# Ulixes-8/UNet-Implementations

Measured on AMD Instinct MI355X. Metric: images/sec (512x512, bs/GPU=8) Our_UNet train step, higher is better.
Workload: dtype f32; 1 GPU; Our_UNet 6-stage 3-class 512x512 bs=8/GPU fp32 train step (fwd + Dice/wCE loss + bwd + SGD-Nesterov), train mode, HIP conv/IN/upsample kernels; global_batch=8, parallelism=dp1, world=1

## Files before the change

include/unet_hip.h:

```cpp
#ifndef UNET_HIP_H_
#define UNET_HIP_H_

#include <stddef.h>
#include <stdint.h>

#ifdef __cplusplus
extern "C" {
#endif

#define UNET_ABI_VERSION 11

#define UNET_OK 0
#define UNET_E_INVALID (-1)
#define UNET_E_LAUNCH (-2)
#define UNET_E_WORKSPACE (-3)

typedef void* unet_stream_t;

const char* unet_last_error(void);
int unet_abi_version(void);
int unet_device_count(void);

int unet_debug_set_chunk_limit(int64_t bytes);

// ... 289 lines not shown
                            size_t workspace_bytes, int N, int H, int W, int Cout,
                            unet_stream_t stream);
int unet_stem_u8_fwd_b16(const uint8_t* image_hwc, const float* mean3, const float* std3,
                         const float* wf, const float* bias, uint16_t* y, void* workspace,
                         size_t workspace_bytes, int* stats_px_out, int N, int H, int W, int Cout,
                         unet_stream_t stream);
int unet_stem_u8_bwd_weight_b16(const uint8_t* image_hwc, const float* mean3, const float* std3,
                                const uint16_t* dy, float* dw_oihw, void* workspace,
                                size_t workspace_bytes, int N, int H, int W, int Cout,
                                unet_stream_t stream);

size_t unet_stem_in_bwd_weight_fold_workspace_bytes(int N, int H, int W, int Cout);
int unet_stem_in_bwd_weight_fold(const float* x, const uint8_t* image_hwc, const float* mean3,
                                 const float* std3, const float* g, const float* y,
                                 const float* mean, const float* rstd, const float* gamma,
                                 const float* beta, const float* mask, float slope,
                                 const void* partial, int tiles, float* dw_oihw, float* dgamma,
                                 float* dbeta, float* dbias, void* workspace,
                                 size_t workspace_bytes, int N, int H, int W, int Cout,
                                 unet_stream_t stream);

int unet_conv_in_bwd_weight_fold32_supported(int N, int H, int W, int Cx, int Cout);
size_t unet_conv_in_bwd_weight_fold32_workspace_bytes(int N, int H, int W);
int unet_conv_in_bwd_weight_fold32(const unet_act_src* x, float slope_x, float* g, const float* y,
                                   const float* mean, const float* rstd, const float* gamma,
                                   const float* beta, const float* mask, float slope,
                                   const void* partial, int tiles, float* dw_oihw, int ci_offset,
                                   int Cin_total, float* dgamma, float* dbeta, float* dbias,
                                   void* workspace, size_t workspace_bytes, int N, int H, int W,
                                   unet_stream_t stream);

int unet_conv_in_bwd_weight(const unet_act_src* x, float slope, const float* dy, float* dw_oihw,
                            int ci_offset, int Cin_total, int ksize, int stride, void* workspace,
                            size_t workspace_bytes, int N, int H, int W, int Cout,
                            unet_stream_t stream);
int unet_conv_in_bwd_weight_bf16x3(const unet_act_src* x, float slope, const float* dy, float* dw_oihw,
                            int ci_offset, int Cin_total, int ksize, int stride, void* workspace,
                            size_t workspace_bytes, int N, int H, int W, int Cout,
                            unet_stream_t stream);

int unet_upsample2x_in_fwd(const unet_act_src* x, float slope, float* up, int N, int h, int w,
                           unet_stream_t stream);

int unet_upsample2x_bwd_taps(const float* dy, float* D, int N, int h, int w, int C,
                             unet_stream_t stream);
int unet_resize_bilinear_fwd(const float* x, float* y, int planes, int h, int w, int H, int W,
                             unet_stream_t stream);
int unet_resize_bilinear_bwd(const float* gy, float* gx, int planes, int h, int w, int H, int W,
                             unet_stream_t stream);
size_t unet_conv3x3_up_bwd_weight_workspace_bytes(int N, int h, int w, int Cx, int Cout);
int unet_conv3x3_up_bwd_weight(const unet_act_src* x, float slope, const float* D, float* dw_oihw,
                               int ci_offset, int Cin_total, void* workspace,
                               size_t workspace_bytes, int N, int h, int w, int Cout,
                               unet_stream_t stream);
int unet_conv3x3_up_bwd_data(const float* D, const float* wd, int Cin_total, int ci_offset,
                             float* g, int N, int h, int w, int Cout, int Ccols, int accumulate,
                             unet_stream_t stream);

typedef struct unet_bwd_stats {
  const float* y;
  const float* mean;
  const float* rstd;
  const float* gamma;
  const float* beta;
  const float* mask;
  float slope;
  void* partial;
  size_t partial_bytes;
  int tiles_out;
} unet_bwd_stats;
int unet_conv3x3_bwd_data_bs(const float* dy, const float* wd, int Cin_total, int ci_offset,
                             float* dx, int N, int H, int W, int Cout, int Ccols, int stride,
                             int accumulate, unet_bwd_stats* bs, unet_stream_t stream);
int unet_conv3x3_bwd_data_bs_b16(const uint16_t* dy, const float* wd, int Cin_total, int ci_offset,
                                 uint16_t* dx, int N, int H, int W, int Cout, int Ccols, int stride,
                                 int accumulate, unet_bwd_stats* bs, unet_stream_t stream);
int unet_conv3x3_bwd_data_bs_bf16x3(const float* dy, const float* wd, const uint16_t* wd3,
                                    int Cin_total, int ci_offset, float* dx, int N, int H, int W,
                                    int Cout, int Ccols, int stride, int accumulate,
                                    unet_bwd_stats* bs, unet_stream_t stream);
int unet_conv3x3_up_bwd_data_bs(const float* D, const float* wd, int Cin_total, int ci_offset,
                                float* g, int N, int h, int w, int Cout, int Ccols, int accumulate,
                                unet_bwd_stats* bs, unet_stream_t stream);
int unet_conv_wino_supported(int N, int H, int W, int C0, int C1, int Cout);
int unet_set_c32_winograd(int on);
int unet_conv_c32_is_winograd(int N, int H, int W, int Cin, int Cout, int stride);
int unet_conv_up_c32_is_winograd(int N, int H, int W, int C0, int C1, int Cout);
size_t unet_wino_weight_floats(int Cout, int Cin);
int unet_pack_wino_weights(const float* w_oihw, float* uf, float* ud, int Cout, int Cin,
                           unet_stream_t stream);
typedef struct unet_wino_pack_entry {
  const float* w;
  float* uf;
  float* ud;
  int Cout, Cin;
  int block_begin, reserved;
} unet_wino_pack_entry;
int unet_pack_wino_weights_batched(const unet_wino_pack_entry* table_device, int n,
                                   int total_blocks, unet_stream_t stream);
int unet_conv_in_fwd_wino(const unet_act_src* s0, const unet_act_src* s1, float slope,
                          const float* uf, const float* bias, float* y, void* workspace,
                          size_t workspace_bytes, int* stats_px_out, int N, int H, int W, int Cout,
                          unet_stream_t stream);
int unet_conv3x3_bwd_weight_is_winograd(int N, int H, int W, int Cx, int Cout, int stride);
int unet_conv_up_wino_supported(int N, int H, int W, int C0, int C1, int Cout);
int unet_conv_up_in_fwd_wino(const unet_act_src* low, const unet_act_src* skip, float slope,
                             const float* uf, const float* bias, float* y, void* workspace,
                             size_t workspace_bytes, int* stats_px_out, int N, int H, int W,
                             int Cout, unet_stream_t stream);
int unet_conv3x3_bwd_data_bs_wino(const float* dy, const float* ud, int Cin_total, int ci_offset,
                                  float* dx, int N, int H, int W, int Cout, int Ccols,
                                  unet_bwd_stats* bs, unet_stream_t stream);

int unet_instnorm_bwd_merge_partials(const void* partial, int tiles, void* coef, void* sums, int N,
                                     int HW, int C, unet_stream_t stream);

int unet_instnorm_lrelu_drop_bwd_partials(const float* ga, const float* y, const float* mean,
                                          const float* rstd, const float* gamma,
                                          const float* beta, const float* mask, float slope,
                                          float* dy, float* dgamma, float* dbeta, float* dbias,
                                          const void* partial, int tiles, void* workspace,
                                          size_t workspace_bytes, int N, int HW, int C,
                                          unet_stream_t stream);
int unet_instnorm_lrelu_drop_bwd_partials_b16(const uint16_t* ga, const uint16_t* y,
                                              const float* mean, const float* rstd,
                                              const float* gamma, const float* beta,
                                              const float* mask, float slope, uint16_t* dy,
                                              float* dgamma, float* dbeta, float* dbias,
                                              const void* partial, int tiles, void* workspace,
                                              size_t workspace_bytes, int N, int HW, int C,
                                              unet_stream_t stream);

int unet_conv_in_fwd_b16(const unet_act_src* s0, const unet_act_src* s1, float slope,
                         const float* w, const float* bias, int ksize, int stride, uint16_t* y,
                         void* workspace, size_t workspace_bytes, int* stats_px_out, int N, int H,
                         int W, int Cout, unet_stream_t stream);
int unet_conv_in_fwd_b16_wb(const unet_act_src* s0, const unet_act_src* s1, float slope,
                            const float* w, const uint16_t* wb, const float* bias, int ksize,
                            int stride, uint16_t* y, void* workspace, size_t workspace_bytes,
                            int* stats_px_out, int N, int H, int W, int Cout, unet_stream_t stream);
int unet_conv3x3_bwd_data_bs_b16_wb(const uint16_t* dy, const float* wd, const uint16_t* wdb,
                                    int Cin_total, int ci_offset, uint16_t* dx, int N, int H,
                                    int W, int Cout, int Ccols, int stride, int accumulate,
                                    unet_bwd_stats* bs, unet_stream_t stream);
int unet_conv_in_stats_finalize_b16(const uint16_t* y, void* workspace, size_t workspace_bytes,
                                    int stats_px, const float* gamma, const float* beta, float eps,
                                    const float* mask, float* mean, float* rstd, float* alpha_out,
                                    float* beta_out, int N, int HoWo, int Cout,
                                    unet_stream_t stream);
int unet_conv_in_bwd_weight_b16(const unet_act_src* x, float slope, const uint16_t* dy,
                                float* dw_oihw, int ci_offset, int Cin_total, int ksize, int stride,
                                void* workspace, size_t workspace_bytes, int N, int H, int W,
                                int Cout, unet_stream_t stream);
int unet_conv3x3_bwd_data_b16(const uint16_t* dy, const float* wd, int Cin_total, int ci_offset,
                              uint16_t* dx, int N, int H, int W, int Cout, int Ccols, int stride,
                              int accumulate, unet_stream_t stream);
int unet_instnorm_lrelu_drop_bwd_b16(const uint16_t* ga, const uint16_t* y, const float* mean,
                                     const float* rstd, const float* gamma, const float* beta,
                                     const float* mask, float slope, uint16_t* dy, float* dgamma,
                                     float* dbeta, float* dbias, void* workspace,
                                     size_t workspace_bytes, int N, int HW, int C,
                                     unet_stream_t stream);
int unet_upsample2x_in_fwd_b16(const unet_act_src* x, float slope, uint16_t* up, int N, int h,
                               int w, unet_stream_t stream);
int unet_conv_up_in_fwd_b16_supported(int N, int H, int W, int C0, int C1, int Cout);
int unet_conv_up_in_fwd_b16(const unet_act_src* low, const unet_act_src* skip, float slope,
// ... 133 lines not shown
```

unet-implementations_amd/_lib.py:

```python
import ctypes
import os
import subprocess

_HERE = os.path.dirname(os.path.abspath(__file__))
LIB_PATH = os.environ.get("UNET_HIP_LIB") or os.path.join(_HERE, "libunet_hip.so")
CSRC = os.path.join(_HERE, "csrc")

ABI_VERSION = 11

_c = ctypes
_p = _c.c_void_p
_i = _c.c_int
_f = _c.c_float
_sz = _c.c_size_t
_i64 = _c.c_int64



class ActSrc(ctypes.Structure):
    _fields_ = [("x", _p), ("C", _i), ("alpha", _p), ("beta", _p)]


_ps = _c.POINTER(ActSrc)

# ... 75 lines not shown
    "unet_augment_post_apply": (_i, [_p, _p, _p, _p, _p, _sz, _i, _i, _i, _p]),
    "unet_augment_light_params_per_sample": (_i, []),
    "unet_augment_light_workspace_bytes": (_sz, [_i]),
    "unet_augment_light_u8": (_i, [_p, _p, _p, _p, _p, _sz, _i, _i, _i, _p]),
    "unet_augment_light_stats": (_i, [_p, _p, _p, _sz, _i, _i, _i, _p]),
    "unet_augment_light_apply": (_i, [_p, _p, _p, _p, _p, _sz, _i, _i, _i, _p]),
    "unet_gradcam_workspace_bytes": (_sz, [_i, _i, _i]),
    "unet_gradcam_weights": (_i, [_p, _i, _p, _p, _sz, _i, _i, _i, _p]),
    "unet_gradcam_map": (_i, [_ps, _i, _f, _p, _p, _p, _sz, _i, _i, _p]),
    "unet_gradcam_heatmap": (_i, [_p, _p, _sz, _p, _i, _i, _i, _i, _i, _p]),
    "unet_preprocess_u8": (_i, [_p, _p, _p, _p, _i, _i, _i, _c.POINTER(_f), _c.POINTER(_f), _p]),
    "unet_sgd_nesterov_step": (_i, [_p, _p, _p, _i64, _f, _f, _f, _i, _f, _p]),
    "unet_sgd_nesterov_step_dev": (_i, [_p, _p, _p, _i64, _p, _i, _p]),
    "unet_conv_in_fwd_workspace_bytes": (_sz, [_i, _i, _i, _i, _i]),
    "unet_conv_in_fwd": (_i, [_ps, _ps, _f, _p, _p, _i, _i, _p, _p, _sz, _c.POINTER(_i), _i, _i, _i,
                              _i, _p]),
    "unet_conv_in_fwd_bf16x3": (_i, [_ps, _ps, _f, _p, _p, _p, _i, _i, _p, _p, _sz, _c.POINTER(_i), _i,
                                     _i, _i, _i, _p]),
    "unet_conv_up_in_fwd_supported": (_i, [_i, _i, _i, _i, _i, _i]),
    "unet_conv_up_in_fwd": (_i, [_ps, _ps, _f, _p, _p, _p, _p, _sz, _c.POINTER(_i), _i, _i, _i, _i,
                                 _p]),
    "unet_conv_in_stats_finalize": (_i, [_p, _p, _sz, _i, _p, _p, _f, _p, _p, _p, _p, _p, _i, _i, _i,
                                         _p]),
    "unet_stem_u8_fwd": (_i, [_p, _c.POINTER(_f), _c.POINTER(_f), _p, _p, _p, _p, _sz,
                              _c.POINTER(_i), _i, _i, _i, _i, _p]),
    "unet_stem_u8_bwd_weight": (_i, [_p, _c.POINTER(_f), _c.POINTER(_f), _p, _p, _p, _sz, _i, _i,
                                     _i, _i, _p]),
    "unet_conv_in_bwd_weight": (_i, [_ps, _f, _p, _p, _i, _i, _i, _i, _p, _sz, _i, _i, _i, _i, _p]),
    "unet_conv_in_bwd_weight_bf16x3": (_i, [_ps, _f, _p, _p, _i, _i, _i, _i, _p, _sz, _i, _i, _i, _i,
                                            _p]),
    "unet_upsample2x_in_fwd": (_i, [_ps, _f, _p, _i, _i, _i, _p]),
    "unet_conv3x3_bwd_data_bs": (_i, [_p, _p, _i, _i, _p, _i, _i, _i, _i, _i, _i, _i, _pbs, _p]),
    "unet_conv_wino_supported": (_i, [_i, _i, _i, _i, _i, _i]),
    "unet_set_c32_winograd": (_i, [_i]),
    "unet_conv_c32_is_winograd": (_i, [_i, _i, _i, _i, _i, _i]),
    "unet_conv_up_c32_is_winograd": (_i, [_i, _i, _i, _i, _i, _i]),
    "unet_wino_weight_floats": (_sz, [_i, _i]),
    "unet_pack_wino_weights": (_i, [_p, _p, _p, _i, _i, _p]),
    "unet_pack_wino_weights_batched": (_i, [_p, _i, _i, _p]),
    "unet_conv_in_fwd_wino": (_i, [_ps, _ps, _f, _p, _p, _p, _p, _sz, _c.POINTER(_i), _i, _i, _i,
                                   _i, _p]),
    "unet_conv3x3_bwd_weight_is_winograd": (_i, [_i, _i, _i, _i, _i, _i]),
    "unet_conv_up_wino_supported": (_i, [_i, _i, _i, _i, _i, _i]),
    "unet_conv_up_in_fwd_wino": (_i, [_ps, _ps, _f, _p, _p, _p, _p, _sz, _c.POINTER(_i), _i, _i,
                                      _i, _i, _p]),
    "unet_conv3x3_bwd_data_bs_wino": (_i, [_p, _p, _i, _i, _p, _i, _i, _i, _i, _i, _pbs, _p]),
    "unet_conv3x3_bwd_data_bs_b16": (_i, [_p, _p, _i, _i, _p, _i, _i, _i, _i, _i, _i, _i, _pbs, _p]),
    "unet_conv3x3_bwd_data_bs_b16_wb": (_i, [_p, _p, _p, _i, _i, _p, _i, _i, _i, _i, _i, _i, _i, _pbs,
                                             _p]),
    "unet_conv3x3_bwd_data_bs_bf16x3": (_i, [_p, _p, _p, _i, _i, _p, _i, _i, _i, _i, _i, _i, _i, _pbs,
                                             _p]),
    "unet_conv3x3_up_bwd_data_bs": (_i, [_p, _p, _i, _i, _p, _i, _i, _i, _i, _i, _i, _pbs, _p]),
    "unet_instnorm_lrelu_drop_bwd_partials": (_i, [_p, _p, _p, _p, _p, _p, _p, _f, _p, _p, _p, _p,
                                                   _p, _i, _p, _sz, _i, _i, _i, _p]),
    "unet_instnorm_lrelu_drop_bwd_partials_b16": (_i, [_p, _p, _p, _p, _p, _p, _p, _f, _p, _p, _p, _p,
                                                       _p, _i, _p, _sz, _i, _i, _i, _p]),
    "unet_conv_in_fwd_b16": (_i, [_ps, _ps, _f, _p, _p, _i, _i, _p, _p, _sz, _c.POINTER(_i), _i, _i,
                                  _i, _i, _p]),
    "unet_conv_in_fwd_b16_wb": (_i, [_ps, _ps, _f, _p, _p, _p, _i, _i, _p, _p, _sz, _c.POINTER(_i),
                                     _i, _i, _i, _i, _p]),
    "unet_conv_in_stats_finalize_b16": (_i, [_p, _p, _sz, _i, _p, _p, _f, _p, _p, _p, _p, _p, _i, _i,
                                             _i, _p]),
    "unet_conv_in_bwd_weight_b16": (_i, [_ps, _f, _p, _p, _i, _i, _i, _i, _p, _sz, _i, _i, _i, _i,
                                         _p]),
    "unet_conv3x3_bwd_data_b16": (_i, [_p, _p, _i, _i, _p, _i, _i, _i, _i, _i, _i, _i, _p]),
    "unet_instnorm_lrelu_drop_bwd_b16": (_i, [_p, _p, _p, _p, _p, _p, _p, _f, _p, _p, _p, _p, _p,
                                              _sz, _i, _i, _i, _p]),
    "unet_upsample2x_in_fwd_b16": (_i, [_ps, _f, _p, _i, _i, _i, _p]),
    "unet_upsample2x_bwd_taps_b16": (_i, [_p, _p, _i, _i, _i, _i, _p]),
    "unet_conv3x3_up_bwd_weight_b16": (_i, [_ps, _f, _p, _p, _i, _i, _p, _sz, _i, _i, _i, _i, _p]),
    "unet_conv_up_in_fwd_b16_supported": (_i, [_i, _i, _i, _i, _i, _i]),
    "unet_conv_up_in_fwd_b16": (_i, [_ps, _ps, _f, _p, _p, _p, _p, _p, _sz, _c.POINTER(_i), _i, _i, _i,
                                     _i, _p]),
    "unet_conv3x3_up_bwd_data_b16": (_i, [_p, _p, _i, _i, _p, _i, _i, _i, _i, _i, _i, _p]),
    "unet_conv3x3_up_bwd_data_bs_b16": (_i, [_p, _p, _i, _i, _p, _i, _i, _i, _i, _i, _i, _pbs, _p]),
    "unet_conv3x3_up_bwd_data_bs_b16_wb": (_i, [_p, _p, _p, _i, _i, _p, _i, _i, _i, _i, _i, _i, _pbs,
                                           _p]),
    "unet_head1x1_in_fwd_b16": (_i, [_ps, _f, _p, _p, _p, _i, _i, _i, _p]),
    "unet_head1x1_in_bwd_b16": (_i, [_ps, _f, _p, _p, _p, _p, _p, _p, _sz, _i, _i, _i, _p]),
    "unet_upsample2x_bwd_taps": (_i, [_p, _p, _i, _i, _i, _i, _p]),
    "unet_conv3x3_up_bwd_weight_workspace_bytes": (_sz, [_i, _i, _i, _i, _i]),
    "unet_conv3x3_up_bwd_weight": (_i, [_ps, _f, _p, _p, _i, _i, _p, _sz, _i, _i, _i, _i, _p]),
    "unet_conv3x3_up_bwd_data": (_i, [_p, _p, _i, _i, _p, _i, _i, _i, _i, _i, _i, _p]),
    "unet_head1x1_in_fwd": (_i, [_ps, _f, _p, _p, _p, _i, _i, _i, _p]),
    "unet_head1x1_in_bwd": (_i, [_ps, _f, _p, _p, _p, _p, _p, _p, _sz, _i, _i, _i, _p]),
    "unet_head1x1_in_bwd_bs": (_i, [_ps, _f, _p, _p, _p, _p, _p, _p, _sz, _i, _i, _i, _pbs, _p]),
    "unet_head1x1_in_bwd_bs_b16": (_i, [_ps, _f, _p, _p, _p, _p, _p, _p, _sz, _i, _i, _i, _pbs, _p]),
    "unet_stem_in_bwd_weight_fold_workspace_bytes": (_sz, [_i, _i, _i, _i]),
    "unet_stem_in_bwd_weight_fold": (_i, [_p, _p, _c.POINTER(_f), _c.POINTER(_f), _p, _p, _p, _p, _p,
                                          _p, _p, _f, _p, _i, _p, _p, _p, _p, _p, _sz, _i, _i, _i,
                                          _i, _p]),
    "unet_conv_in_bwd_weight_fold32_supported": (_i, [_i, _i, _i, _i, _i]),
    "unet_conv_in_bwd_weight_fold32_workspace_bytes": (_sz, [_i, _i, _i]),
    "unet_conv_in_bwd_weight_fold32": (_i, [_ps, _f, _p, _p, _p, _p, _p, _p, _p, _f, _p, _i, _p, _i,
                                            _i, _p, _p, _p, _p, _sz, _i, _i, _i, _p]),
    "unet_instnorm_bwd_merge_partials": (_i, [_p, _i, _p, _p, _i, _i, _i, _p]),
    "unet_head1x1_in_bwd_fold_workspace_bytes": (_sz, [_i, _i, _i]),
    "unet_head1x1_in_bwd_fold": (_i, [_ps, _f, _p, _p, _p, _p, _p, _p, _p, _p, _p, _sz, _i, _i, _i,
                                      _pbs, _p]),
    "unet_recon3x3_fwd": (_i, [_ps, _i, _f, _p, _p, _p, _i, _i, _i, _i, _p]),
    "unet_recon3x3_bwd_workspace_bytes": (_sz, [_i, _i, _i]),
    "unet_recon3x3_bwd": (_i, [_ps, _i, _f, _p, _p, _p, _p, _p, _p, _p, _sz, _i, _i, _i, _i, _pbs,
                               _p]),
    "unet_mse_loss_workspace_bytes": (_sz, [_i, _i, _i, _i]),
    "unet_mse_loss_fwd": (_i, [_p, _p, _i, _p, _p, _p, _sz, _i, _i, _i, _i, _p]),
    "unet_mse_loss_grad": (_i, [_p, _p, _i, _p, _p, _i, _i, _i, _i, _p]),
    "unet_adam_step": (_i, [_p, _p, _p, _p, _i64, _p, _i, _p]),
    "unet_ssim_workspace_bytes": (_sz, [_i, _i, _i, _i]),
    "unet_ssim_fwd": (_i, [_p, _p, _i, _c.POINTER(_f), _f, _f, _p, _p, _p, _c.c_double,
                           _c.c_double, _p, _sz, _i, _i, _i, _i, _p]),
    "unet_ssim_grad": (_i, [_p, _p, _i, _c.POINTER(_f), _f, _f, _p, _i, _c.c_double, _c.c_double,
                            _p, _i, _i, _i, _i, _p]),
    "unet_perceptual_prep": (_i, [_p, _p, _i, _c.POINTER(_f), _c.POINTER(_f), _p, _i, _i, _i, _p]),
    "unet_relu_maxpool2x2_fwd": (_i, [_p, _p, _i, _i, _i, _i, _p]),
    "unet_feature_mse_workspace_bytes": (_sz, [_i, _i, _i, _i]),
    "unet_feature_mse_fwd": (_i, [_p, _p, _p, _sz, _i, _i, _i, _i, _p]),
    "unet_perceptual_relu_bwd": (_i, [_p, _p, _f, _p, _p, _p, _i, _i, _i, _i, _p]),
    "unet_perceptual_stem_bwd_data": (_i, [_p, _p, _c.POINTER(_f), _p, _i, _i, _i, _i, _p]),
    "unet_vit_patchify": (_i, [_p, _i, _c.POINTER(_f), _c.POINTER(_f), _p, _i, _i, _i, _i, _i, _i,
                               _p]),
    "unet_vit_gemm_bf16": (_i, [_p, _p, _p, _p, _i, _i, _i, _i, _p]),
    "unet_vit_tokens_ln": (_i, [_p, _p, _p, _p, _p, _f, _p, _i, _i, _i, _p]),
    "unet_vit_layernorm": (_i, [_p, _p, _p, _f, _p, _i, _i, _p]),
    "unet_vit_attention": (_i, [_p, _p, _i, _i, _i, _i, _p]),
    "unet_vit_head": (_i, [_p, _p, _p, _f, _p, _p, _i, _i, _i, _i, _i, _p]),
    "unet_stem_u8_fwd_b16": (_i, [_p, _c.POINTER(_f), _c.POINTER(_f), _p, _p, _p, _p, _sz,
                                  _c.POINTER(_i), _i, _i, _i, _i, _p]),
    "unet_stem_u8_bwd_weight_b16": (_i, [_p, _c.POINTER(_f), _c.POINTER(_f), _p, _p, _p, _sz, _i,
                                         _i, _i, _i, _p]),
}
for _name in ("unet_dice_wce_loss_fwd_bwd", "unet_dice_wce_loss_grad",
              "unet_dice_wce_loss_shard_stats", "unet_dice_wce_loss_shard_apply",
              "unet_argmax_dice_counts"):
    SIGNATURES[_name + "_u8"] = SIGNATURES[_name]
del _name

_lib = None


class UNetHipError(RuntimeError):
    pass


def build(verbose=False):
    jobs = str(min(8, os.cpu_count() or 1))
    proc = subprocess.run(["make", "-C", CSRC, "-j", jobs], capture_output=True, text=True)
    if verbose or proc.returncode != 0:
        print(proc.stdout)
        print(proc.stderr)
    if proc.returncode != 0:
        raise UNetHipError("building libunet_hip.so failed (see output above)")
    return LIB_PATH


def lib():
    global _lib
    if _lib is not None:
        return _lib
    if not os.path.exists(LIB_PATH):
        raise UNetHipError(
            f"{LIB_PATH} is missing: run `python -c 'import __graft_entry__ as g; g.build()'` "
            "(there is no CPU / eager fallback for the HIP path)")
    import torch
    handle = ctypes.CDLL(LIB_PATH, mode=ctypes.RTLD_GLOBAL)
    for name, (res, args) in SIGNATURES.items():
        fn = getattr(handle, name)
# ... 13 lines not shown
```

unet-implementations_amd/csrc/conv_igemm.hip:

```cpp
#include "conv_host.h"

namespace unet_conv {
namespace {


template <int BM, int BN, int WM, int WN, int BK, bool FUSED = false, int KG = 1>
__global__ __launch_bounds__(256 * KG, KG == 1 ? 2 : 1) void conv_igemm_kernel(const IgemmParams p) {
  constexpr int LDA = BK + 4;
  constexpr int SEGS = BK / 4;
  constexpr int ROWS = 256 / SEGS;
  constexpr int TM = WM / 32, TN = WN / 32;
  constexpr int WAVES_N = BN / WN;
  static_assert((BM / WM) * (BN / WN) == 4, "4 waves per block");
  constexpr int A_PASSES = BM / ROWS;
  constexpr int B_PASSES = BN / ROWS;
  constexpr int A_TILE = BM * LDA, B_TILE = BN * LDA;
  extern __shared__ __attribute__((aligned(16))) float smem[];
  const int grp = KG > 1 ? __builtin_amdgcn_readfirstlane((int)(threadIdx.x >> 8)) : 0;
  const bool lead = KG == 1 || grp == 0;
  float* As = smem + grp * 2 * (A_TILE + B_TILE);
  float* Bs = As + 2 * A_TILE;

  const int tid = threadIdx.x & 255, lane = tid & 63, wave = tid >> 6;
  const int li = lane & 31, lh = lane >> 5;
  const int wm0 = (wave / WAVES_N) * WM, wn0 = (wave % WAVES_N) * WN;

  const int tiles_n = p.Ncols / BN;
  const int bid = xcd_remap(blockIdx.x, gridDim.x);
  const int tm = bid / tiles_n, tn = bid - tm * tiles_n;
  const int m0 = tm * BM, n0 = tn * BN;
  const int HlWl = p.Hl * p.Wl;
  const int M = p.N * HlWl;
  const int Ktot = p.C0 + p.C1;

  const int lrow = tid / SEGS, lseg = tid % SEGS;
  int a_nb[A_PASSES], a_iy[A_PASSES], a_ix[A_PASSES];
  int a_img[FUSED ? A_PASSES : 1];
#pragma unroll
  for (int i = 0; i < A_PASSES; ++i) {
    const int m = m0 + lrow + ROWS * i;
    if (m < M) {
      const int n = m / HlWl;
      const int r = m - n * HlWl;
      const int a = r / p.Wl;
      const int b = r - a * p.Wl;
      a_nb[i] = n * p.Hin * p.Win;
      a_iy[i] = a * p.sin;
      a_ix[i] = b * p.sin;
      if (FUSED) a_img[i] = n;
    } else {
      a_nb[i] = 0;
      a_iy[i] = -(1 << 24);
      a_ix[i] = 0;
      if (FUSED) a_img[i] = 0;
    }
  }
  const __amdgpu_buffer_rsrc_t rs0 = __builtin_amdgcn_make_buffer_rsrc(
      const_cast<float*>(p.src0), 0, (int)p.src0_bytes, 0x00020000);
  const __amdgpu_buffer_rsrc_t rs1 = __builtin_amdgcn_make_buffer_rsrc(
      const_cast<float*>(p.src1 ? p.src1 : p.src0), 0, (int)p.src1_bytes, 0x00020000);
  const __amdgpu_buffer_rsrc_t rsw = __builtin_amdgcn_make_buffer_rsrc(
      const_cast<float*>(p.w), 0, (int)p.w_bytes, 0x00020000);
  const unsigned wrow_off = (unsigned)((p.n_off + n0 + lrow) * Ktot + lseg * 4) * 4u;

  typedef int i32x4 __attribute__((ext_vector_type(4)));
  f32x4 ra[A_PASSES], rb[B_PASSES];
  f32x16 acc[TM][TN];
#pragma unroll
  for (int m = 0; m < TM; ++m)
#pragma unroll
    for (int n = 0; n < TN; ++n)
#pragma unroll
      for (int r = 0; r < 16; ++r) acc[m][n][r] = 0.f;

  const int KS = p.ntaps * (Ktot / BK) / KG;

  constexpr int CP = FUSED ? A_PASSES : 1;
  f32x4 ca[CP], cb[CP];
  float cs = 1.f;
  unsigned okm = 0;
  auto load_tiles = [&](int t, int chunk) {
    const unsigned tw = (t < 4) ? p.tapw[0] : (t < 8 ? p.tapw[1] : p.tapw[2]);
    const unsigned e = (tw >> ((t & 3) * 8)) & 0xffu;
    const int oy = (int)(e & 3u) - 1, ox = (int)((e >> 2) & 3u) - 1;
    const int wt = (int)(e >> 4);
    const int c = chunk * BK;
    const bool first = c < p.C0;
    const __amdgpu_buffer_rsrc_t rs = first ? rs0 : rs1;
    const int Cs = first ? (p.src0_pitch ? p.src0_pitch : p.C0) : p.C1;
    const int coff = (first ? c : c - p.C0) + lseg * 4 + wt * p.tap_cstride;
    if (FUSED) {
      const float* al = first ? p.act0_alpha : p.act1_alpha;
      const float* be = first ? p.act0_beta : p.act1_beta;
      if (al) {
#pragma unroll
        for (int i = 0; i < CP; ++i) {
          ca[i] = *reinterpret_cast<const f32x4*>(al + (size_t)a_img[i] * Cs + coff);
          cb[i] = *reinterpret_cast<const f32x4*>(be + (size_t)a_img[i] * Cs + coff);
        }
        cs = p.slope;
      } else {
#pragma unroll
        for (int i = 0; i < CP; ++i) {
          ca[i] = f32x4{1.f, 1.f, 1.f, 1.f};
          cb[i] = f32x4{0.f, 0.f, 0.f, 0.f};
        }
        cs = 1.f;
      }
      okm = 0;
    }
#pragma unroll
    for (int i = 0; i < A_PASSES; ++i) {
      const int iy = a_iy[i] + oy, ix = a_ix[i] + ox;
      const bool ok = (unsigned)iy < (unsigned)p.Hin && (unsigned)ix < (unsigned)p.Win;
      if (FUSED) okm |= (ok ? 1u : 0u) << i;
      const unsigned off = ((unsigned)((a_nb[i] + iy * p.Win + ix) * Cs + coff) * 4u) |
                           (ok ? 0u : 0x80000000u);
      const i32x4 v = __builtin_amdgcn_raw_buffer_load_b128(rs, off, 0, 0);
      ra[i] = __builtin_bit_cast(f32x4, v);
    }
    const unsigned woff = wrow_off + (unsigned)(wt * p.tap_stride + c) * 4u;
#pragma unroll
    for (int j = 0; j < B_PASSES; ++j) {
      const i32x4 v = __builtin_amdgcn_raw_buffer_load_b128(rsw, woff + (unsigned)(ROWS * j * Ktot) * 4u, 0, 0);
      rb[j] = __builtin_bit_cast(f32x4, v);
    }
  };
  auto store_tiles = [&](int buf) {
    float* Ab = As + buf * A_TILE + lrow * LDA + lseg * 4;
    float* Bb = Bs + buf * B_TILE + lrow * LDA + lseg * 4;
#pragma unroll
    for (int i = 0; i < A_PASSES; ++i) {
      if (FUSED) ra[i] = act4(ra[i], ca[i], cb[i], cs, (okm >> i) & 1u);
      *reinterpret_cast<f32x4*>(Ab + ROWS * i * LDA) = ra[i];
    }
#pragma unroll
    for (int j = 0; j < B_PASSES; ++j) *reinterpret_cast<f32x4*>(Bb + ROWS * j * LDA) = rb[j];
  };

  int t_next = 0, chunk_next = 0;
  if (KG > 1) {
    chunk_next = grp * KS / p.ntaps;
    t_next = grp * KS - chunk_next * p.ntaps;
  }
  auto advance = [&](bool on) {
    const int tn = t_next + 1;
    const bool wrap = tn == p.ntaps;
    t_next = on ? (wrap ? 0 : tn) : t_next;
    chunk_next = on ? chunk_next + (wrap ? 1 : 0) : chunk_next;
  };

  load_tiles(t_next, chunk_next);
  advance(KS > 1);
  store_tiles(0);
  __syncthreads();

  const int frag_off = li * LDA + 4 * lh;
  for (int ks = 0; ks < KS; ++ks) {
    const int buf = ks & 1;
    load_tiles(t_next, chunk_next);
    advance(ks + 2 < KS);
    const float* Ab = As + buf * A_TILE + wm0 * LDA + frag_off;
    const float* Bb = Bs + buf * B_TILE + wn0 * LDA + frag_off;
    f32x4 a[2][TM], b[2][TN];
#pragma unroll
    for (int m = 0; m < TM; ++m) a[0][m] = *reinterpret_cast<const f32x4*>(Ab + m * 32 * LDA);
#pragma unroll
    for (int n = 0; n < TN; ++n) b[0][n] = *reinterpret_cast<const f32x4*>(Bb + n * 32 * LDA);
#pragma unroll
    for (int kk = 0; kk < BK / 8; ++kk) {
      const int cur = kk & 1, nxt = cur ^ 1;
      if (kk + 1 < BK / 8) {
#pragma unroll
        for (int m = 0; m < TM; ++m)
          a[nxt][m] = *reinterpret_cast<const f32x4*>(Ab + m * 32 * LDA + (kk + 1) * 8);
#pragma unroll
        for (int n = 0; n < TN; ++n)
          b[nxt][n] = *reinterpret_cast<const f32x4*>(Bb + n * 32 * LDA + (kk + 1) * 8);
      }
#pragma unroll
      for (int r = 0; r < 4; ++r)
#pragma unroll
        for (int m = 0; m < TM; ++m)
#pragma unroll
          for (int n = 0; n < TN; ++n)
            acc[m][n] = __builtin_amdgcn_mfma_f32_32x32x2f32(a[cur][m][r], b[cur][n][r], acc[m][n],
                                                             0, 0, 0);
    }
    if (!FUSED) store_tiles(buf ^ 1);
    if (BK / 8 > 1) __builtin_amdgcn_sched_group_barrier(0x100, 2 * (TM + TN), 0);
    else __builtin_amdgcn_sched_group_barrier(0x100, TM + TN, 0);
    __builtin_amdgcn_sched_group_barrier(0x008, 4 * TM * TN, 0);
    __builtin_amdgcn_sched_group_barrier(0x020, A_PASSES + B_PASSES, 0);
#pragma unroll
    for (int kk = 1; kk < BK / 8; ++kk) {
      if (kk + 1 < BK / 8) __builtin_amdgcn_sched_group_barrier(0x100, TM + TN, 0);
      __builtin_amdgcn_sched_group_barrier(0x008, 4 * TM * TN, 0);
    }
    if (FUSED) {
      __builtin_amdgcn_sched_barrier(0);
// ... 1311 lines not shown
  return UNET_OK;
}

extern "C" int unet_conv_in_fwd(const unet_act_src* s0, const unet_act_src* s1, float slope,
                                const float* w, const float* bias, int ksize, int stride, float* y,
                                void* workspace, size_t workspace_bytes, int* stats_px_out, int N,
                                int H, int W, int Cout, unet_stream_t stream) {
  return conv_in_fwd_impl(s0, s1, slope, w, bias, ksize, stride, y, workspace, workspace_bytes,
                          stats_px_out, N, H, W, Cout, ConvMode::f32(), (hipStream_t)stream);
}

extern "C" int unet_conv_in_fwd_bf16x3(const unet_act_src* s0, const unet_act_src* s1, float slope,
                                       const float* w, const uint16_t* w3, const float* bias,
                                       int ksize, int stride, float* y, void* workspace,
                                       size_t workspace_bytes, int* stats_px_out, int N, int H,
                                       int W, int Cout, unet_stream_t stream) {
  UNET_REQUIRE(w3 || ksize != 3, "conv_in_fwd_bf16x3: the pre-split weight planes are null");
  return conv_in_fwd_impl(s0, s1, slope, w, bias, ksize, stride, y, workspace, workspace_bytes,
                          stats_px_out, N, H, W, Cout, ConvMode::split(w3), (hipStream_t)stream);
}

extern "C" int unet_conv_in_fwd_b16(const unet_act_src* s0, const unet_act_src* s1, float slope,
                                    const float* w, const float* bias, int ksize, int stride,
                                    uint16_t* y, void* workspace, size_t workspace_bytes,
                                    int* stats_px_out, int N, int H, int W, int Cout,
                                    unet_stream_t stream) {
  return conv_in_fwd_impl(s0, s1, slope, w, bias, ksize, stride, y, workspace, workspace_bytes,
                          stats_px_out, N, H, W, Cout, ConvMode::b16(nullptr), (hipStream_t)stream);
}

extern "C" int unet_conv_in_fwd_b16_wb(const unet_act_src* s0, const unet_act_src* s1,
                                       float slope, const float* w, const uint16_t* wb,
                                       const float* bias, int ksize, int stride, uint16_t* y,
                                       void* workspace, size_t workspace_bytes, int* stats_px_out,
                                       int N, int H, int W, int Cout, unet_stream_t stream) {
  return conv_in_fwd_impl(s0, s1, slope, w, bias, ksize, stride, y, workspace, workspace_bytes,
                          stats_px_out, N, H, W, Cout, ConvMode::b16(ksize == 3 ? wb : nullptr),
                          (hipStream_t)stream);
}

static int conv_in_stats_finalize_impl(const void* y, void* workspace, size_t workspace_bytes,
                                       int stats_px, const float* gamma, const float* beta,
                                       float eps, const float* mask, float* mean, float* rstd,
                                       float* alpha_out, float* beta_out, int N, int HoWo, int Cout,
                                       unet_stream_t stream, Elem elem) {
  UNET_REQUIRE(y && workspace && mean && rstd, "conv_in_stats_finalize: null pointer");
  UNET_REQUIRE(stats_px >= 0 && (stats_px == 0 || HoWo % stats_px == 0),
               "conv_in_stats_finalize: %d-pixel tiles do not cover %d pixels", stats_px, HoWo);
  if (stats_px > 0)
    return unet_in_finalize_tiles(workspace, HoWo / stats_px, stats_px, gamma, beta, eps, mask,
                                  mean, rstd, alpha_out, beta_out, N, HoWo, Cout,
                                  (hipStream_t)stream,
                                  reinterpret_cast<char*>(workspace) +
                                      stats_partial_bytes(N, HoWo, Cout));
  return unet_in_stats_masked(static_cast<const float*>(y), gamma, beta, eps, mask, mean, rstd,
                              alpha_out, beta_out, workspace, workspace_bytes, N, HoWo, Cout,
                              (hipStream_t)stream, elem == Elem::BF16);
}

extern "C" int unet_conv_in_stats_finalize(const float* y, void* workspace, size_t workspace_bytes,
                                           int stats_px, const float* gamma, const float* beta,
                                           float eps, const float* mask, float* mean, float* rstd,
                                           float* alpha_out, float* beta_out, int N, int HoWo,
                                           int Cout, unet_stream_t stream) {
  return conv_in_stats_finalize_impl(y, workspace, workspace_bytes, stats_px, gamma, beta, eps,
                                     mask, mean, rstd, alpha_out, beta_out, N, HoWo, Cout, stream,
                                     Elem::F32);
}

extern "C" int unet_conv_in_stats_finalize_b16(const uint16_t* y, void* workspace,
                                               size_t workspace_bytes, int stats_px,
                                               const float* gamma, const float* beta, float eps,
                                               const float* mask, float* mean, float* rstd,
                                               float* alpha_out, float* beta_out, int N, int HoWo,
                                               int Cout, unet_stream_t stream) {
  return conv_in_stats_finalize_impl(y, workspace, workspace_bytes, stats_px, gamma, beta, eps,
                                     mask, mean, rstd, alpha_out, beta_out, N, HoWo, Cout, stream,
                                     Elem::BF16);
}

static int conv3x3_up_bwd_data_impl(const void* D, const float* wd, int Cin_total, int ci_offset,
                                    void* g, int N, int h, int w, int Cout, int Ccols,
                                    int accumulate, const ConvMode& m, unet_bwd_stats* bs,
                                    hipStream_t stream) {
  if (bs) bs->tiles_out = 0;
  UNET_REQUIRE(D && wd && g, "conv3x3_up_bwd_data: null pointer");
  UNET_REQUIRE(Cout > 0 && Cout % 32 == 0 && Ccols > 0 && Ccols % 32 == 0 && ci_offset >= 0 &&
                   ci_offset + Ccols <= Cin_total && N > 0 && h > 0 && w > 0,
               "conv3x3_up_bwd_data: bad shape Cout=%d Ccols=%d slice %d of %d", Cout, Ccols,
               ci_offset, Cin_total);
  UNET_REQUIRE((long long)9 * Cout * Cin_total * 4 < (1LL << 31),
               "conv3x3_up_bwd_data: weights exceed 2 GiB");
  const long long D_image = (long long)h * w * 9 * Cout * (long long)m.es();
  return for_each_chunk("conv3x3_up_bwd_data", N, D_image, [&](Batch b) {
    BsBinder bsb(b.whole(bs), true, N, h * w, Ccols);
    IgemmParams p = dgrad_params(D, wd, Cin_total, ci_offset, g, b, h, w, Cout, Ccols, 1, 3,
                                 accumulate, true, m);
    bsb.bind(p);
    const int rc = m.b16_tensors() ? dispatch_igemm_b16(p, stream, nullptr, bsb.report())
                                   : dispatch_igemm(p, stream, nullptr, bsb.report());
    return bsb.done_px(rc, h * w);
  });
}

extern "C" int unet_conv3x3_up_bwd_data_bs(const float* D, const float* wd, int Cin_total,
                                           int ci_offset, float* g, int N, int h, int w, int Cout,
                                           int Ccols, int accumulate, unet_bwd_stats* bs,
                                           unet_stream_t stream) {
  return conv3x3_up_bwd_data_impl(D, wd, Cin_total, ci_offset, g, N, h, w, Cout, Ccols, accumulate,
                                  ConvMode::f32(), bs, (hipStream_t)stream);
}

extern "C" int unet_conv3x3_up_bwd_data(const float* D, const float* wd, int Cin_total,
                                        int ci_offset, float* g, int N, int h, int w, int Cout,
                                        int Ccols, int accumulate, unet_stream_t stream) {
  return conv3x3_up_bwd_data_impl(D, wd, Cin_total, ci_offset, g, N, h, w, Cout, Ccols, accumulate,
                                  ConvMode::f32(), nullptr, (hipStream_t)stream);
}

extern "C" int unet_conv3x3_up_bwd_data_b16(const uint16_t* D, const float* wd, int Cin_total,
                                            int ci_offset, uint16_t* g, int N, int h, int w,
                                            int Cout, int Ccols, int accumulate,
                                            unet_stream_t stream) {
  return conv3x3_up_bwd_data_impl(D, wd, Cin_total, ci_offset, g, N, h, w, Cout, Ccols, accumulate,
                                  ConvMode::b16(nullptr), nullptr, (hipStream_t)stream);
}

extern "C" int unet_conv3x3_up_bwd_data_bs_b16_wb(const uint16_t* D, const float* wd,
                                                  const uint16_t* wdb, int Cin_total,
                                                  int ci_offset, uint16_t* g, int N, int h, int w,
                                                  int Cout, int Ccols, int accumulate,
                                                  unet_bwd_stats* bs, unet_stream_t stream) {
  return conv3x3_up_bwd_data_impl(D, wd, Cin_total, ci_offset, g, N, h, w, Cout, Ccols, accumulate,
                                  ConvMode::b16(wdb), bs, (hipStream_t)stream);
}

extern "C" int unet_conv3x3_up_bwd_data_bs_b16(const uint16_t* D, const float* wd, int Cin_total,
                                               int ci_offset, uint16_t* g, int N, int h, int w,
                                               int Cout, int Ccols, int accumulate,
                                               unet_bwd_stats* bs, unet_stream_t stream) {
  return conv3x3_up_bwd_data_impl(D, wd, Cin_total, ci_offset, g, N, h, w, Cout, Ccols, accumulate,
                                  ConvMode::b16(nullptr), bs, (hipStream_t)stream);
}

template <typename TO>
static int stem_u8_fwd_impl(const uint8_t* image_hwc, const float* mean3, const float* std3,
                            const float* wf, const float* bias, TO* y, void* workspace,
                            size_t workspace_bytes, int* stats_px_out, int N, int H, int W,
                            int Cout, hipStream_t stream) {
  UNET_REQUIRE(image_hwc && mean3 && std3 && wf && y && workspace && stats_px_out,
               "stem_u8_fwd: null pointer");
  UNET_REQUIRE(N > 0 && H > 0 && W > 0 && W % STEM_ROW_PIX == 0 && Cout > 0 && Cout % 32 == 0,
               "stem_u8_fwd: needs W %% %d == 0 and Cout %% 32 == 0 (got W=%d Cout=%d)",
               STEM_ROW_PIX, W, Cout);
  if (workspace_bytes < unet_conv_in_fwd_workspace_bytes(N, H, W, Cout, 1)) {
    unet_set_error("stem_u8_fwd: workspace too small");
    return UNET_E_WORKSPACE;
  }
  StemNorm nm;
  for (int c = 0; c < 3; ++c) { nm.mean[c] = mean3[c]; nm.std[c] = std3[c]; }
  launch_stem_fwd_rows<unsigned char, TO>(image_hwc, wf, bias, y, N, H, W, Cout,
                                          reinterpret_cast<float2*>(workspace), nm, stream);
  UNET_CHECK_LAUNCH("conv_stem_fwd(u8)");
  *stats_px_out = STEM_ROW_PIX;
  return UNET_OK;
}

extern "C" int unet_stem_u8_fwd(const uint8_t* image_hwc, const float* mean3, const float* std3,
                                const float* wf, const float* bias, float* y, void* workspace,
                                size_t workspace_bytes, int* stats_px_out, int N, int H, int W,
                                int Cout, unet_stream_t stream) {
  return stem_u8_fwd_impl(image_hwc, mean3, std3, wf, bias, y, workspace, workspace_bytes,
                          stats_px_out, N, H, W, Cout, (hipStream_t)stream);
}

extern "C" int unet_stem_u8_fwd_b16(const uint8_t* image_hwc, const float* mean3,
                                    const float* std3, const float* wf, const float* bias,
                                    uint16_t* y, void* workspace, size_t workspace_bytes,
                                    int* stats_px_out, int N, int H, int W, int Cout,
                                    unet_stream_t stream) {
  return stem_u8_fwd_impl(image_hwc, mean3, std3, wf, bias, reinterpret_cast<__bf16*>(y), workspace,
                          workspace_bytes, stats_px_out, N, H, W, Cout, (hipStream_t)stream);
}

extern "C" int unet_conv_up_in_fwd_supported(int N, int H, int W, int C0, int C1, int Cout) {
  if (N <= 0 || H <= 0 || W <= 0 || H % 4 || W % 32 || C0 < 32 || C0 % 32 || C1 < 0 || C1 % 32 ||
      Cout % 32)
    return 0;
  const long long M = (long long)N * H * W, mt = M / 128;
  if ((long long)H * W * (C0 > 4 * C1 ? C0 / 4 : C1) * 4 * N >= (1LL << 31)) return 0;
  if (Cout % 128 == 0 && mt * (Cout / 128) >= 512) return 1;
  if (Cout % 64 == 0 && mt * (Cout / 64) >= 512) return 1;
  if (Cout == 32 && H % 8 == 0 && M / 256 >= 512) return 1;
  if (Cout == 32 && C0 == 64 && C1 == 32 && H % 8 == 0 && c32_winograd_flag() == 2) return 1;
  return 0;
}

extern "C" int unet_conv_up_in_fwd_b16_supported(int N, int H, int W, int C0, int C1, int Cout) {
  if (N <= 0 || H <= 0 || W <= 0 || H % 4 || W % 32 || C0 < 32 || C0 % 32 || C1 < 0 || C1 % 32 ||
      Cout % 32)
// ... 77 lines not shown
```

unet-implementations_amd/csrc/conv_params.h:

```cpp
#pragma once
#include "common.h"

namespace unet_conv {

struct IgemmParams {
  const float* src0;
  const float* src1;
  int C0, C1;
  const float* w;
  int tap_stride;
  int n_off;
  unsigned src0_bytes, src1_bytes, w_bytes;
  const float* bias;
  float* out;
  int ldo;
  int accumulate;
  int N, Hin, Win;
  int Hl, Wl;
  int Hout, Wout;
  int sin;
  int sout, py, px;
  int ntaps;
  unsigned tapw[3];
  int Ncols;
  const __bf16* w3;
  int w3_plane;
  unsigned w3_bytes;
  const float* act0_alpha; const float* act0_beta;
  const float* act1_alpha; const float* act1_beta;
  float slope;
  float2* stats;
  int stats_tiles;
  int tap_cstride;
  int src0_pitch;
  const float* bs_y;
  const float* bs_mean;
  const float* bs_rstd;
  const float* bs_gamma;
  const float* bs_beta;
  const float* bs_mask;
  float2* bs_partial;
  int bs_tiles;
  int bs_tile0;
};

long long& chunk_limit_bytes();
inline int batch_chunk(int N, long long per_image_bytes) {
  const long long lim = chunk_limit_bytes();
  const long long n = lim / (per_image_bytes > 0 ? per_image_bytes : 1);
  return (int)(n < N ? n : N);
}

constexpr int kNoTileFits = 1;

inline int deep_k_groups(const IgemmParams& p) {
  const long long M = (long long)p.N * p.Hl * p.Wl;
  if (p.Ncols % 64 != 0 || ceil_div64(M, 64) * (p.Ncols / 64) > 256) return 1;
  const int ks = p.ntaps * ((p.C0 + p.C1) / 32);
  int kg = 4;
  while (kg > 1 && (ks % kg != 0 || ks / kg < 4)) kg >>= 1;
  return kg;
}

inline void set_tap(IgemmParams& p, int t, int oy, int ox, int wt) {
  const unsigned e = (unsigned)(oy + 1) | ((unsigned)(ox + 1) << 2) | ((unsigned)wt << 4);
  p.tapw[t >> 2] |= e << ((t & 3) * 8);
}

#ifdef __HIPCC__
template <typename TO>
__device__ __forceinline__ void store_block16(TO* const (&o)[16], const f32x16& acc, float bv,
                                              int accumulate) {
  if (accumulate) {
    float old[16];
#pragma unroll
    for (int r = 0; r < 16; ++r) old[r] = o[r] ? ld1(o[r]) : 0.f;
#pragma unroll
    for (int r = 0; r < 16; ++r)
      if (o[r]) st1(o[r], acc[r] + bv + old[r]);
  } else {
#pragma unroll
    for (int r = 0; r < 16; ++r)
      if (o[r]) st1(o[r], acc[r] + bv);
  }
}
constexpr unsigned kNoOut = 0xffffffffu;
template <typename TO>
__device__ __forceinline__ void store_block16_off(TO* base, const unsigned (&o)[16],
                                                  const f32x16& acc, float bv, int accumulate) {
  if (accumulate) {
    float old[16];
#pragma unroll
    for (int r = 0; r < 16; ++r) old[r] = o[r] != kNoOut ? ld1(base + o[r]) : 0.f;
#pragma unroll
    for (int r = 0; r < 16; ++r)
      if (o[r] != kNoOut) st1(base + o[r], acc[r] + bv + old[r]);
  } else {
#pragma unroll
    for (int r = 0; r < 16; ++r)
      if (o[r] != kNoOut) st1(base + o[r], acc[r] + bv);
  }
}
#endif

#ifdef __HIPCC__
typedef float f32x2 __attribute__((ext_vector_type(2)));
__device__ __forceinline__ f32x4 act4f(const f32x4 v, const f32x4 al, const f32x4 be,
                                       float slope, float okf) {
  const f32x4 z = (v * al + be) * okf;
  const f32x4 sz = z * slope;
  return __builtin_elementwise_max(z, sz);
}
__device__ __forceinline__ f32x4 act4(const f32x4 v, const f32x4 al, const f32x4 be, float slope,
                                      bool ok) {
  return act4f(v, al, be, slope, ok ? 1.f : 0.f);
}

// ... 119 lines not shown
```

unet-implementations_amd/csrc/conv_wgrad.hip:

```cpp
#include "conv_params.h"
#include <vector>
#include "lds_asm.h"
#include <type_traits>
#include <utility>

namespace {
using unet_conv::act4;
using unet_conv::act4f;
template <int I> using template_ic = std::integral_constant<int, I>;
template <int B, int... I, typename F>
__device__ __forceinline__ void for_range_impl(std::integer_sequence<int, I...>, F&& f) {
  (f(template_ic<B + I>{}), ...);
}
template <int B, int E, typename F>
__device__ __forceinline__ void for_range(F&& f) {
  for_range_impl<B>(std::make_integer_sequence<int, (E > B ? E - B : 0)>{}, f);
}

struct WgradParams {
  const float* x;
  const float* dy;
  float* partial;
  int Cx, Cout;
  int N, H, W, Ho, Wo;
  int segs_per_row, total_segs, segs_per_block, split;
  int ci_tiles, co_tiles;
  unsigned x_bytes, dy_bytes;
  const float* alpha;
  const float* beta;
  float slope;
  int b16;
  const float* fy; const float* fmu; const float* frstd; const float* fgamma; const float* fbeta;
  const float* fmask; const float2* fcoef; const float2* fsums;
  float* fdgamma; float* fdbeta; float* fdbias;
  float fslope;
};

template <int NSB, int NPP, int TJ, int NT, typename ACC>
__device__ __forceinline__ void wgrad_epilogue(float* smem, const WgradParams& p, int sp, int ci0,
                                               int co0, int sb, int pp, ACC&& acc_of) {
  const int tid = threadIdx.x, lane = tid & 63;
  {
    constexpr int TPR = 3;
    const f32x4* M4 = reinterpret_cast<const f32x4*>(smem);
    for_range<0, 3>([&](auto uc) {
      constexpr int u = decltype(uc)::value;
      for_range<0, TPR>([&](auto vc) {
        constexpr int v = decltype(vc)::value;
        const f32x16& a = acc_of(template_ic<u * 3 + v>{});
        float* dst = smem + ((v * NPP + pp) * NSB + sb) * 1024 + lane;
#pragma unroll
        for (int r = 0; r < 16; ++r) dst[r * 64] = a[r];
      });
      __syncthreads();
      for (int i = tid; i < TPR * NSB * 256; i += NT) {
        const int v = i / (NSB * 256), rem = i - v * (NSB * 256);
        const int s = rem >> 8, e4 = rem & 255;
        f32x4 sum = M4[((v * NPP) * NSB + s) * 256 + e4];
#pragma unroll
        for (int q = 1; q < NPP; ++q) sum += M4[((v * NPP + q) * NSB + s) * 256 + e4];
        const int r = e4 >> 4, l0 = (e4 & 15) * 4;
        const int row = (r & 3) + 8 * (r >> 2) + 4 * (l0 >> 5);
        const int swi = s / TJ, swj = s - swi * TJ;
        float* out = p.partial +
            ((size_t)(sp * 9 + u * 3 + v) * p.Cx + ci0 + swi * 32 + row) * p.Cout +
            co0 + swj * 32 + (l0 & 31);
        *reinterpret_cast<f32x4*>(out) = sum;
      }
      __syncthreads();
    });
  }
}
constexpr size_t kWgradMergeLds4 = (size_t)3 * 4 * 1024 * sizeof(float);
constexpr size_t kWgradMergeLds8 = (size_t)3 * 8 * 1024 * sizeof(float);

template <int CI_T, int CO_T, int S, int STRIDE, bool ACT = false, typename TX = float,
          typename TD = float, int NW = 4>
__global__ __launch_bounds__(64 * NW, 2) void conv_wgrad_kernel(const WgradParams p) {
  constexpr int TI = CI_T / 32, TJ = CO_T / 32;
  constexpr int NSB = TI * TJ, NPP = NW / NSB;
  static_assert(NSB == 1 || NSB == 2 || NSB == 4, "tile must have 1, 2 or 4 sub-blocks");
  static_assert(NW == 4 || NW == 8, "4 or 8 waves");
  constexpr int NT = 64 * NW;
  constexpr int PW = (S - 1) * STRIDE + 3;
  constexpr int NP4 = 3 * PW * CI_T / 4;
  constexpr int ND4 = S * CO_T / 4;
  constexpr int PATCH = NP4 * 4;
  constexpr int STAGE = PATCH + ND4 * 4;
  constexpr int NLP = (NP4 + NT - 1) / NT, NLD = (ND4 + NT - 1) / NT;
  constexpr int NQ = (S / 2) / NPP;
  extern __shared__ __attribute__((aligned(16))) float smem[];

  const int tid = threadIdx.x, lane = tid & 63, wave = tid >> 6;
  const int li = lane & 31, lh = lane >> 5;
  const int sb = wave % NSB, pp = wave / NSB;
  const int wi = sb / TJ, wj = sb - wi * TJ;

  int bid = blockIdx.x;
  const int co_t = bid % p.co_tiles; bid /= p.co_tiles;
  const int ci_t = bid % p.ci_tiles; bid /= p.ci_tiles;
  const int sp = bid;
  const int ci0 = ci_t * CI_T, co0 = co_t * CO_T;
  const int g_begin = sp * p.segs_per_block;
  const int g_end = min(g_begin + p.segs_per_block, p.total_segs);

  const __amdgpu_buffer_rsrc_t rsx = __builtin_amdgcn_make_buffer_rsrc(
      const_cast<float*>(p.x), 0, (int)p.x_bytes, 0x00020000);
  const __amdgpu_buffer_rsrc_t rsd = __builtin_amdgcn_make_buffer_rsrc(
      const_cast<float*>(p.dy), 0, (int)p.dy_bytes, 0x00020000);

  int p_rc[NLP];
  const int p_ch = ci0 + (tid % (CI_T / 4)) * 4;
#pragma unroll
  for (int k = 0; k < NLP; ++k) {
// ... 96 lines not shown
      float* nxt_stage = smem + (buf ^ 1) * STAGE;
      float a[2][3][3], b[2];
      {
        const int xx = 2 * pp + lh;
#pragma unroll
        for (int u = 0; u < 3; ++u)
#pragma unroll
          for (int v = 0; v < 3; ++v) a[0][u][v] = P[(u * PW + xx * STRIDE + v) * CI_T];
        b[0] = D[xx * CO_T];
      }
      for_range<0, NQ>([&](auto qc) {
        constexpr int q = decltype(qc)::value;
        constexpr int cur = q & 1, nxt = cur ^ 1;
        if constexpr (q + 1 < NQ) {
          const int xx = 2 * (pp + NPP * (q + 1)) + lh;
#pragma unroll
          for (int u = 0; u < 3; ++u)
#pragma unroll
            for (int v = 0; v < 3; ++v) a[nxt][u][v] = P[(u * PW + xx * STRIDE + v) * CI_T];
          b[nxt] = D[xx * CO_T];
        }
#pragma unroll
        for (int u = 0; u < 3; ++u)
#pragma unroll
          for (int v = 0; v < 3; ++v)
            acc[u][v] = __builtin_amdgcn_mfma_f32_32x32x2f32(a[cur][u][v], b[cur], acc[u][v], 0, 0, 0);
        if constexpr (q < LQ)
          for_range<q * LPER, ((q + 1) * LPER < NLS ? (q + 1) * LPER : NLS)>(issue_slot);
        if constexpr (q >= NQ - HALF) {
          constexpr int s0 = (q - (NQ - HALF)) * APER;
          for_range<s0, (s0 + APER < NLS ? s0 + APER : NLS)>(
              [&](auto kc) { put_slot(kc, nxt_stage); });
        }
        __builtin_amdgcn_sched_barrier(0);
      });
      __syncthreads();
    }
  }

  wgrad_epilogue<NSB, NPP, TJ, NT>(smem, p, sp, ci0, co0, sb, pp, [&](auto tc) -> const f32x16& {
    constexpr int t = decltype(tc)::value;
    return acc[t / 3][t % 3];
  });
}

template <int CI_T, int CO_T, int S, bool ACT, typename TX = float, typename TD = float,
          int NW = 4>
__global__ __launch_bounds__(64 * NW, 2) void conv_wgrad_taps_kernel(const WgradParams p) {
  constexpr int TI = CI_T / 32, TJ = CO_T / 32;
  constexpr int NSB = TI * TJ, NPP = NW / NSB;
  static_assert(NSB == 1 || NSB == 2 || NSB == 4, "tile must have 1, 2 or 4 sub-blocks");
  constexpr int NT = 64 * NW;
  constexpr int BW = 9 * CO_T;
  constexpr int NA4 = S * CI_T / 4;
  constexpr int NB4 = S * BW / 4;
  constexpr int ATILE = NA4 * 4;
  constexpr int STAGE = ATILE + NB4 * 4;
  constexpr int NLA = (NA4 + NT - 1) / NT, NLB = (NB4 + NT - 1) / NT;
  static_assert(NA4 % NT == 0 || NLA == 1, "A slots");
  static_assert(NB4 % NT == 0, "D slots fill whole passes");
  constexpr int NQ = (S / 2) / NPP;
  extern __shared__ __attribute__((aligned(16))) float smem[];

  const int tid = threadIdx.x, lane = tid & 63, wave = tid >> 6;
  const int li = lane & 31, lh = lane >> 5;
  const int sb = wave % NSB, pp = wave / NSB;
  const int wi = sb / TJ, wj = sb - wi * TJ;

  int bid = xcd_remap(blockIdx.x, gridDim.x);
  const int co_t = bid % p.co_tiles; bid /= p.co_tiles;
  const int ci_t = bid % p.ci_tiles; bid /= p.ci_tiles;
  const int sp = bid;
  const int ci0 = ci_t * CI_T, co0 = co_t * CO_T;
  const int g_begin = sp * p.segs_per_block;
  const int g_end = min(g_begin + p.segs_per_block, p.total_segs);
  const int HW = p.H * p.W;
  const int Q = p.N * HW;

  const __amdgpu_buffer_rsrc_t rsx = __builtin_amdgcn_make_buffer_rsrc(
      const_cast<float*>(p.x), 0, (int)p.x_bytes, 0x00020000);
  const __amdgpu_buffer_rsrc_t rsd = __builtin_amdgcn_make_buffer_rsrc(
      const_cast<float*>(p.dy), 0, (int)p.dy_bytes, 0x00020000);

  int a_px[NLA];
  unsigned b_off[NLB];
  const int a_ch = ci0 + (tid % (CI_T / 4)) * 4;
#pragma unroll
  for (int k = 0; k < NLA; ++k) a_px[k] = (tid + NT * k) / (CI_T / 4);
#pragma unroll
  for (int k = 0; k < NLB; ++k) {
    const int idx = tid + NT * k;
    const int px = idx / (BW / 4);
    const int f = (idx - px * (BW / 4)) * 4;
    const int t = f / CO_T;
    b_off[k] = (unsigned)(px * (9 * p.Cout) + t * p.Cout + co0 + (f - t * CO_T));
  }

  f32x4 ra[NLA], rb[NLB];
  f32x4 ca[NLA], cb[NLA];
  unsigned okm = 0;
  int lq0 = 0;
  auto issue_slot = [&](auto kc) {
    constexpr int k = decltype(kc)::value;
    if constexpr (k < NLA) {
      const int q = lq0 + a_px[k];
      const bool ok = q < Q && (NA4 % NT == 0 || tid < NA4);
      ra[k] = buf_ld4<TX>(rsx, (unsigned)(q * p.Cx + a_ch), ok ? 0u : 0x80000000u);
      if (ACT) {
        const int n = ok ? q / HW : 0;
        ca[k] = *reinterpret_cast<const f32x4*>(p.alpha + (size_t)n * p.Cx + a_ch);
        cb[k] = *reinterpret_cast<const f32x4*>(p.beta + (size_t)n * p.Cx + a_ch);
        okm |= (ok ? 1u : 0u) << k;
      }
    } else {
      constexpr int j = k - NLA;
      rb[j] = buf_ld4<TD>(rsd, (unsigned)(lq0 * (9 * p.Cout)) + b_off[j], 0u);
    }
  };
  auto act_slot = [&](auto kc) {
    constexpr int k = decltype(kc)::value;
    if (ACT) ra[k] = act4(ra[k], ca[k], cb[k], p.slope, (okm >> k) & 1u);
  };
  auto store_stage = [&](int buf) {
    float* base = smem + buf * STAGE;
#pragma unroll
    for (int k = 0; k < NLA; ++k)
      if (NA4 % NT == 0 || tid < NA4) *reinterpret_cast<f32x4*>(base + 4 * (tid + NT * k)) = ra[k];
#pragma unroll
    for (int k = 0; k < NLB; ++k)
      *reinterpret_cast<f32x4*>(base + ATILE + 4 * (tid + NT * k)) = rb[k];
  };

  f32x16 acc[9];
#pragma unroll
  for (int t = 0; t < 9; ++t)
#pragma unroll
    for (int r = 0; r < 16; ++r) acc[t][r] = 0.f;

  constexpr int NLS = NLA + NLB;
  constexpr int LQ = NQ >= 4 ? NQ / 2 : 1;
  constexpr int LPER = (NLS + LQ - 1) / LQ;

  if (g_begin < g_end) {
    lq0 = g_begin * S;
    for_range<0, NLS>(issue_slot);
    for_range<0, NLA>(act_slot);
    store_stage(0);
    __syncthreads();
    for (int g = g_begin; g < g_end; ++g) {
      const int buf = (g - g_begin) & 1;
      if (g + 1 < g_end) lq0 += S;
      okm = 0;
      const float* A = smem + buf * STAGE + wi * 32 + li;
      const float* B = smem + buf * STAGE + ATILE + wj * 32 + li;
      float a[2], b[2][9];
      {
        const int xx = 2 * pp + lh;
        a[0] = A[xx * CI_T];
#pragma unroll
        for (int t = 0; t < 9; ++t) b[0][t] = B[xx * BW + t * CO_T];
      }
      for_range<0, NQ>([&](auto qc) {
        constexpr int q = decltype(qc)::value;
        constexpr int cur = q & 1, nxt = cur ^ 1;
        if constexpr (q + 1 < NQ) {
          const int xx = 2 * (pp + NPP * (q + 1)) + lh;
          a[nxt] = A[xx * CI_T];
#pragma unroll
          for (int t = 0; t < 9; ++t) b[nxt][t] = B[xx * BW + t * CO_T];
        }
#pragma unroll
        for (int t = 0; t < 9; ++t)
          acc[t] = __builtin_amdgcn_mfma_f32_32x32x2f32(a[cur], b[cur][t], acc[t], 0, 0, 0);
        if constexpr (q < LQ)
          for_range<q * LPER, ((q + 1) * LPER < NLS ? (q + 1) * LPER : NLS)>(issue_slot);
        if constexpr (ACT && q == NQ - 1) for_range<0, NLA>(act_slot);
        __builtin_amdgcn_sched_barrier(0);
      });
      store_stage(buf ^ 1);
      __syncthreads();
    }
  }

  wgrad_epilogue<NSB, NPP, TJ, NT>(smem, p, sp, ci0, co0, sb, pp, [&](auto tc) -> const f32x16& {
    return acc[decltype(tc)::value];
  });
}

template <int CI_T, int CO_T, int S, bool ACT>
__global__ __launch_bounds__(256, 2) void conv_wgrad_taps_b16_kernel(const WgradParams p) {
  constexpr int TI = CI_T / 32, TJ = CO_T / 32;
  constexpr int NSB = TI * TJ, NPP = 4 / NSB;
  static_assert(NSB == 1 || NSB == 2 || NSB == 4, "tile must have 1, 2 or 4 sub-blocks");
  constexpr int NT = 256;
  constexpr int SUB = S * 32;
  constexpr int ATILE = TI * SUB, DTILE = 9 * TJ * SUB, STAGE = ATILE + DTILE;
  constexpr int NA = S * CI_T / 4;
  constexpr int ND = S * 9 * CO_T / 8;
  constexpr int NLA = (NA + NT - 1) / NT, NLD = (ND + NT - 1) / NT;
  constexpr int NG = (S / 16) / NPP;
  static_assert((S / 16) % NPP == 0 && NG >= 1, "segment must split into whole k-groups");
  extern __shared__ __attribute__((aligned(16))) __bf16 smem_h[];

  const int tid = threadIdx.x, lane = tid & 63, wave = tid >> 6;
  const int sb = wave % NSB, pp = wave / NSB;
  const int wi = sb / TJ, wj = sb - wi * TJ;

  int bid = xcd_remap(blockIdx.x, gridDim.x);
  const int co_t = bid % p.co_tiles; bid /= p.co_tiles;
  const int ci_t = bid % p.ci_tiles; bid /= p.ci_tiles;
  const int sp = bid;
  const int ci0 = ci_t * CI_T, co0 = co_t * CO_T;
  const int g_begin = sp * p.segs_per_block;
  const int g_end = min(g_begin + p.segs_per_block, p.total_segs);
  const int HW = p.H * p.W;
  const int Q = p.N * HW;

  const __amdgpu_buffer_rsrc_t rsx = __builtin_amdgcn_make_buffer_rsrc(
      const_cast<float*>(p.x), 0, (int)p.x_bytes, 0x00020000);
  const __amdgpu_buffer_rsrc_t rsd = __builtin_amdgcn_make_buffer_rsrc(
      const_cast<float*>(p.dy), 0, (int)p.dy_bytes, 0x00020000);

  int a_px[NLA], a_lds[NLA];
  const int a_seg = tid % (CI_T / 4);
  const int a_ch = ci0 + a_seg * 4;
#pragma unroll
  for (int k = 0; k < NLA; ++k) {
    a_px[k] = (tid + NT * k) / (CI_T / 4);
    a_lds[k] = (a_seg >> 3) * SUB + a_px[k] * 32 + (a_seg & 7) * 4;
  }
  unsigned d_off[NLD];
  int d_lds[NLD];
#pragma unroll
  for (int k = 0; k < NLD; ++k) {
// ... 1822 lines not shown
  if (pl.ci_t == 64 && p.b16) return launch_wgrad_taps_b16<64, 64, 16>(p, stream);
  if (pl.ci_t == 32 && pl.co_t == 32 && p.b16) return launch_wgrad_taps_b16<32, 32, 64>(p, stream);
  if (pl.ci_t == 64) return launch_wgrad_taps<64, 64, 16>(p, stream);
  if (pl.co_t == 64) return launch_wgrad_taps<32, 64, 16>(p, stream);
  return launch_wgrad_taps<32, 32, 32>(p, stream);
}

int launch_wgrad_plan(const WgradParams& p, const WgradPlan& pl, int stride, int prec,
                      hipStream_t stream) {
  if (pl.nw == 8) {
    if (pl.ci_t == 32 && pl.co_t == 32)
      return stride == 1 ? launch_wgrad8_s<32, 32, 1>(p, pl.S, stream)
                         : launch_wgrad8_s<32, 32, 2>(p, pl.S, stream);
    if (pl.ci_t == 32)
      return stride == 1 ? launch_wgrad8_s<32, 64, 1>(p, pl.S, stream)
                         : launch_wgrad8_s<32, 64, 2>(p, pl.S, stream);
    return stride == 1 ? launch_wgrad8_s<64, 64, 1>(p, pl.S, stream)
                       : launch_wgrad8_s<64, 64, 2>(p, pl.S, stream);
  }
  const bool use_bf16 = prec != 0 && stride == 1 && (pl.S / 16) % pl.npp == 0 && pl.S >= 16;
  if (use_bf16 && prec == 3) {
    if (pl.ci_t == 32 && pl.co_t == 32) return launch_wgrad_bf16<32, 32, 64, 3, true>(p, stream);
    if (pl.ci_t == 32) return launch_wgrad_bf16<32, 64, 32, 3>(p, stream);
    return launch_wgrad_bf16<64, 64, 16, 3>(p, stream);
  }
  if (p.b16 && prec == 1 && stride == 2 && (pl.S / 16) % pl.npp == 0 &&
      wgrad_ring_ok(p, pl.rg)) {
    if (pl.ci_t == 64 && pl.S == 16) return launch_wgrad_b16_ring<64, 64, 16, 2>(p, pl.rg, stream);
    if (pl.ci_t == 32 && pl.co_t == 64 && pl.S == 32) return launch_wgrad_b16_ring<32, 64, 32, 2>(p, pl.rg, stream);
  }
  if (p.b16 && prec == 1 && stride == 2 && (pl.S / 16) % pl.npp == 0) {
    if (pl.ci_t == 64 && pl.S == 16) return launch_wgrad_b16<64, 64, 16, 2>(p, stream);
    if (pl.ci_t == 32 && pl.co_t == 64 && pl.S == 32) return launch_wgrad_b16<32, 64, 32, 2>(p, stream);
  }
  if (use_bf16 && prec == 1 && wgrad_ring_ok(p, pl.rg)) {
    if (pl.ci_t == 32 && pl.co_t == 32 && pl.S == 64) return launch_wgrad_b16_ring<32, 32, 64>(p, pl.rg, stream);
    if (pl.ci_t == 32 && pl.co_t == 64 && pl.S == 32) return launch_wgrad_b16_ring<32, 64, 32>(p, pl.rg, stream);
    if (pl.ci_t == 64 && pl.S == 32) return launch_wgrad_b16_ring<64, 64, 32>(p, pl.rg, stream);
    if (pl.ci_t == 64 && pl.S == 16) return launch_wgrad_b16_ring<64, 64, 16>(p, pl.rg, stream);
  }
  if (use_bf16 && prec == 1) {
    if (pl.ci_t == 32 && pl.co_t == 32) return launch_wgrad_bf16<32, 32, 64>(p, stream);
    if (pl.ci_t == 32) return launch_wgrad_bf16<32, 64, 32>(p, stream);
    return pl.S == 32 ? launch_wgrad_bf16<64, 64, 32>(p, stream)
                      : launch_wgrad_bf16<64, 64, 16>(p, stream);
  }
  if (pl.ci_t == 32 && pl.co_t == 32) {
    if (stride == 1)
      return pl.S == 64 ? launch_wgrad<32, 32, 64, 1>(p, stream)
           : pl.S == 32 ? launch_wgrad<32, 32, 32, 1>(p, stream)
                        : launch_wgrad<32, 32, 16, 1>(p, stream);
    return pl.S == 32 ? launch_wgrad<32, 32, 32, 2>(p, stream)
                      : launch_wgrad<32, 32, 16, 2>(p, stream);
  }
  if (pl.ci_t == 32 && pl.co_t == 64) {
    if (stride == 1)
      return pl.S == 32 ? launch_wgrad<32, 64, 32, 1>(p, stream)
                        : launch_wgrad<32, 64, 16, 1>(p, stream);
    return pl.S == 32 ? launch_wgrad<32, 64, 32, 2>(p, stream)
                      : launch_wgrad<32, 64, 16, 2>(p, stream);
  }
  if (stride == 1)
    return pl.S == 32 ? launch_wgrad<64, 64, 32, 1>(p, stream)
                      : launch_wgrad<64, 64, 16, 1>(p, stream);
  return launch_wgrad<64, 64, 16, 2>(p, stream);
}

enum WgradForm { WF_STEM, WF_WINO, WF_WINO32, WF_DIRECT, WF_TAPS };

struct WgradCall {
  const void* x = nullptr;
  const unsigned char* x_u8 = nullptr;
  const float* u8_mean_std = nullptr;
  const void* dy = nullptr;
  const StemNormW* stem_fold = nullptr;
  const StemNormW* fold32 = nullptr;
  const float* alpha = nullptr;
  const float* beta = nullptr;
  float slope = 0.f;
  bool b16 = false;
  int prec = 0;
  bool center_only = false;
  bool taps = false;
  float* dw = nullptr;
  int ci_offset = 0, Cin_total = 0;
  float* db = nullptr;
  void* workspace = nullptr;
  size_t workspace_bytes = 0;
  int N = 0, H = 0, W = 0, Cx = 0, Cout = 0, stride = 1;

  int Ho() const { return (H - 1) / stride + 1; }
  int Wo() const { return (W - 1) / stride + 1; }
  int dy_channels() const { return taps ? 9 * Cout : Cout; }
};

struct WgradSel {
  WgradForm form;
  PlanOpts opt;
  int nmax;
};

int wgrad_batch_chunk(const WgradCall& c) {
  const long long a = (long long)c.H * c.W * c.Cx * 4;
  const long long b = (long long)c.Ho() * c.Wo() * c.dy_channels() * 4;
  return unet_conv::batch_chunk(c.N, a > b ? a : b);
}

WgradSel wgrad_select(const WgradCall& c, int c32) {
  WgradSel s{};
  s.nmax = wgrad_batch_chunk(c);
  const bool fp32 = c.prec == 0 && !c.b16;
  s.opt.wide = fp32 && c.Cx != 3 && wgrad_tile(c.Cx, c.Cout).tiles >= 4;
  if (c.taps) {
    s.form = WF_TAPS;
    s.opt.taps_b16 = c.b16;
    return s;
  }
  if (c.Cx == 3) {
    s.form = WF_STEM;
    return s;
  }
  s.opt.prec = c.stride == 1 ? c.prec : 0;
  s.opt.ring_s2 = c.b16 && c.prec == 1 && c.stride == 2;
  s.opt.ring8 = c.b16 && (s.opt.prec == 1 || s.opt.ring_s2) && c.Cx % 64 == 0 && c.Cout % 64 == 0;
  const bool wino_able = fp32 && !c.center_only && s.nmax >= c.N;
  s.form = wino_able && wgrad_wino32_ok(c.N, c.H, c.W, c.Cx, c.Cout, c.stride, c32) ? WF_WINO32
         : wino_able && wgrad_wino_ok(c.N, c.H, c.W, c.Cx, c.Cout, c.stride)        ? WF_WINO
                                                                                     : WF_DIRECT;
  return s;
}

WgradPlan wgrad_plan(const WgradCall& c, WgradForm form, const PlanOpts& o, int nc) {
  switch (form) {
    case WF_STEM: return make_plan_stem(nc, c.H, c.W, c.Cout);
    case WF_WINO: return make_plan_wino(nc, c.H, c.W, c.Cx, c.Cout);
    case WF_WINO32: return make_plan_wino32(nc, c.H, c.W);
    case WF_TAPS: return make_plan_taps((long long)nc * c.H * c.W, c.Cx, c.Cout, o);
    default: return make_plan(nc, c.H, c.W, c.Cx, c.Cout, c.stride, o);
  }
}

size_t wgrad_ws_floats(const WgradCall& c, const WgradSel& s) {
  PlanOpts o = s.opt;
  o.ring8 = o.ring_s2 = o.taps_b16 = false;
  if (s.form == WF_STEM) return wgrad_plan(c, s.form, o, c.N).ws_floats;
  size_t slabs = 0;
  for (int nb = 0; nb < c.N && s.nmax >= 1; nb += s.nmax)
    slabs += (size_t)wgrad_plan(c, s.form, o, c.N - nb < s.nmax ? c.N - nb : s.nmax).split;
  return slab_ws_floats(slabs, (size_t)9 * c.Cx * c.Cout);
}

int wgrad_launch_chunks(const WgradCall& c, const WgradSel& s, float* ws, int* nslab,
                        hipStream_t stream) {
  const long long es = c.b16 ? 2 : 4;
  const size_t E = (size_t)9 * c.Cx * c.Cout;
  const size_t x_img = (size_t)c.H * c.W * c.Cx * es;
  const size_t dy_img = (size_t)c.Ho() * c.Wo() * c.dy_channels() * es;
  *nslab = 0;
  for (int nb = 0; nb < c.N; nb += s.nmax) {
    const int nc = c.N - nb < s.nmax ? c.N - nb : s.nmax;
    const WgradPlan pl = wgrad_plan(c, s.form, s.opt, nc);
    WgradParams p{};
    p.x = reinterpret_cast<const float*>(static_cast<const char*>(c.x) + nb * x_img);
    p.dy = reinterpret_cast<const float*>(static_cast<const char*>(c.dy) + nb * dy_img);
    p.b16 = c.b16;
    p.partial = ws + (size_t)*nslab * E; p.Cx = c.Cx; p.Cout = c.Cout;
    p.N = nc; p.H = c.H; p.W = c.W; p.Ho = c.Ho(); p.Wo = c.Wo();
    p.segs_per_row = pl.segs_per_row; p.total_segs = pl.total_segs;
    p.segs_per_block = pl.segs_per_block; p.split = pl.split;
    p.ci_tiles = c.Cx / pl.ci_t; p.co_tiles = c.Cout / pl.co_t;
    p.x_bytes = (unsigned)(nc * x_img);
    p.dy_bytes = (unsigned)(nc * dy_img);
    p.alpha = c.alpha ? c.alpha + (size_t)nb * c.Cx : nullptr;
    p.beta = c.alpha ? c.beta + (size_t)nb * c.Cx : nullptr;
    p.slope = c.slope;
    if (c.fold32) {
      UNET_REQUIRE(s.form == WF_WINO32 && nc == c.N, "conv_in_bwd_weight_fold32: not a shape of "
                   "the 32-channel Winograd weight gradient");
      const StemNormW& f = *c.fold32;
      p.fy = f.y; p.fmu = f.mu; p.frstd = f.rstd; p.fgamma = f.gamma; p.fbeta = f.beta;
      p.fmask = f.mask; p.fcoef = f.coef; p.fsums = f.sums;
      p.fdgamma = f.dgamma; p.fdbeta = f.dbeta; p.fdbias = f.dbias; p.fslope = f.slope;
    }
    const int rc = s.form == WF_WINO32 ? launch_wgrad_wino32(p, stream)
                   : s.form == WF_WINO ? launch_wgrad_wino(p, stream)
                   : s.form == WF_TAPS ? launch_wgrad_taps_plan(p, pl, stream)
                                       : launch_wgrad_plan(p, pl, c.stride, c.prec, stream);
    if (rc != UNET_OK) return rc;
    *nslab += pl.split;
  }
  return UNET_OK;
}

int launch_wgrad_stem(const WgradCall& c, const WgradPlan& pl, float* ws, hipStream_t stream) {
  StemNormW nm{};
  if (c.stem_fold) {
    UNET_REQUIRE(c.W % SW_PIX == 0 && !c.b16, "stem_in_bwd_weight_fold: needs W %% %d == 0 and an "
                 "fp32 gradient", SW_PIX);
    nm = *c.stem_fold;
  }
  if (c.x_u8) {
    UNET_REQUIRE(c.W % SW_PIX == 0, "stem_u8_bwd_weight: needs W %% %d == 0", SW_PIX);
    for (int k = 0; k < 3; ++k) { nm.mean[k] = c.u8_mean_std[k]; nm.std[k] = c.u8_mean_std[3 + k]; }
  }
  const dim3 grid(pl.stem_blocks, c.Cout / 32);
  return with_bools(c.x_u8 != nullptr, c.b16, [&](auto u8, auto b16) {
    using TX = std::conditional_t<decltype(u8)::value, unsigned char, float>;
    using TD = std::conditional_t<decltype(b16)::value, __bf16, float>;
    const TX* x = decltype(u8)::value ? reinterpret_cast<const TX*>(c.x_u8)
                                      : static_cast<const TX*>(c.x);
    const TD* dy = static_cast<const TD*>(c.dy);
    if constexpr (!decltype(u8)::value)
      if (c.W % SW_PIX != 0)
        return launch_kernel<conv_stem_wgrad_kernel<TD>>("conv_stem_wgrad", grid, 256, 0, stream, x,
                                                         dy, ws, c.N, c.H, c.W, c.Cout, pl.stem_spb,
                                                         pl.stem_stages);
    return launch_kernel<conv_stem_wgrad_rows_kernel<TX, TD>>("conv_stem_wgrad", grid, 256, 0,
                                                              stream, x, dy, ws, c.N, c.H, c.W,
                                                              c.Cout, pl.stem_spb, pl.stem_stages, nm);
  });
}


__global__ __launch_bounds__(256) void bias_grad_kernel(const float* __restrict__ dy,
                                                        float* __restrict__ out, long long M,
                                                        int C, long long rows_per_chunk) {
  __shared__ float red[8][33];
  const int c = blockIdx.x * 32 + (threadIdx.x & 31);
  const int r = threadIdx.x >> 5;
  const long long m0 = (long long)blockIdx.y * rows_per_chunk;
  const long long m1 = m0 + rows_per_chunk < M ? m0 + rows_per_chunk : M;
  float s = 0.f;
  for (long long m = m0 + r; m < m1; m += 8) s += dy[(size_t)m * C + c];
  red[r][threadIdx.x & 31] = s;
  __syncthreads();
  if (r == 0) {
    float t = 0.f;
#pragma unroll
    for (int k = 0; k < 8; ++k) t += red[k][threadIdx.x];
    out[(size_t)blockIdx.y * C + c] = t;
  }
}

}

extern "C" size_t unet_conv3x3_bwd_weight_workspace_bytes(int N, int H, int W, int Cx, int Cout,
                                                          int stride) {
  if (N <= 0 || H <= 0 || W <= 0 || Cx <= 0 || Cout <= 0) return 0;
  static constexpr struct { bool b16; int prec; bool center_only; int c32; } kRequests[] = {
      {false, 0, false, 0}, {false, 0, false, 2}, {false, 0, true, 0}, {false, 3, false, 0},
      {false, 1, false, 0}, {true, 0, false, 0},  {true, 1, false, 0}};
  size_t m = 0;
  for (const auto& r : kRequests) {
    WgradCall c;
    c.N = N; c.H = H; c.W = W; c.Cx = Cx; c.Cout = Cout; c.stride = stride;
    c.b16 = r.b16; c.prec = r.prec; c.center_only = r.center_only;
    const size_t f = wgrad_ws_floats(c, wgrad_select(c, r.c32));
    if (f > m) m = f;
// ... 246 lines not shown
                       image_hwc ? mean3[2] : 0.f, image_hwc ? std3[0] : 1.f,
                       image_hwc ? std3[1] : 1.f, image_hwc ? std3[2] : 1.f};
  WgradCall c;
  c.x = x; c.x_u8 = image_hwc; c.u8_mean_std = ms; c.dy = g; c.stem_fold = &f;
  c.dw = dw_oihw; c.Cin_total = 3;
  c.workspace = ws + 2 * coef_b; c.workspace_bytes = workspace_bytes - 2 * coef_b;
  c.N = N; c.H = H; c.W = W; c.Cx = 3; c.Cout = Cout;
  return conv_bwd_weight_impl(c, (hipStream_t)stream);
}

extern "C" int unet_conv_in_bwd_weight_fold32_supported(int N, int H, int W, int Cx, int Cout) {
  if (N <= 0 || H <= 0 || W <= 0 || Cx != 32 || Cout != 32) return 0;
  WgradCall c;
  c.N = N; c.H = H; c.W = W; c.Cx = Cx; c.Cout = Cout;
  return wgrad_select(c, unet_conv::c32_winograd_flag()).form == WF_WINO32 ? 1 : 0;
}

extern "C" size_t unet_conv_in_bwd_weight_fold32_workspace_bytes(int N, int H, int W) {
  if (N <= 0 || H <= 0 || W <= 0) return 0;
  return 2 * align_up((size_t)N * 32 * sizeof(float2), 256) +
         unet_conv3x3_bwd_weight_workspace_bytes(N, H, W, 32, 32, 1);
}

extern "C" int unet_conv_in_bwd_weight_fold32(const unet_act_src* x, float slope_x, float* g,
                                              const float* y, const float* mean, const float* rstd,
                                              const float* gamma, const float* beta,
                                              const float* mask, float slope, const void* partial,
                                              int tiles, float* dw_oihw, int ci_offset,
                                              int Cin_total, float* dgamma, float* dbeta,
                                              float* dbias, void* workspace, size_t workspace_bytes,
                                              int N, int H, int W, unet_stream_t stream) {
  const int rc0 = check_conv_in("conv_in_bwd_weight_fold32", x, 3, 1);
  if (rc0 != UNET_OK) return rc0;
  UNET_REQUIRE(g && y && mean && rstd && gamma && beta && partial && tiles > 0 && workspace,
               "conv_in_bwd_weight_fold32: null pointer");
  UNET_REQUIRE(unet_conv_in_bwd_weight_fold32_supported(N, H, W, x->C, 32),
               "conv_in_bwd_weight_fold32: N=%d H=%d W=%d Cx=%d is not a shape of the 32-channel "
               "Winograd weight gradient", N, H, W, x->C);
  UNET_REQUIRE(x->x != g && x->x != y, "conv_in_bwd_weight_fold32: g is rewritten in place and "
               "cannot be the layer's operand");
  const size_t coef_b = align_up((size_t)N * 32 * sizeof(float2), 256);
  if (workspace_bytes < 2 * coef_b) {
    unet_set_error("conv_in_bwd_weight_fold32: workspace too small");
    return UNET_E_WORKSPACE;
  }
  char* ws = reinterpret_cast<char*>(workspace);
  StemNormW f{};
  f.y = y; f.mu = mean; f.rstd = rstd; f.gamma = gamma; f.beta = beta; f.mask = mask;
  f.coef = reinterpret_cast<const float2*>(ws);
  f.sums = reinterpret_cast<const float2*>(ws + coef_b);
  f.dgamma = dgamma; f.dbeta = dbeta; f.dbias = dbias; f.slope = slope;
  const int rc = unet_instnorm_bwd_merge_partials(partial, tiles, ws, ws + coef_b, N, H * W, 32,
                                                  stream);
  if (rc != UNET_OK) return rc;
  WgradCall c;
  set_source(c, x, slope_x);
  c.dy = g; c.fold32 = &f;
  c.dw = dw_oihw; c.ci_offset = ci_offset; c.Cin_total = Cin_total;
  c.workspace = ws + 2 * coef_b; c.workspace_bytes = workspace_bytes - 2 * coef_b;
  c.N = N; c.H = H; c.W = W; c.Cout = 32;
  return conv_bwd_weight_impl(c, (hipStream_t)stream);
}

extern "C" size_t unet_conv3x3_up_bwd_weight_workspace_bytes(int N, int h, int w, int Cx, int Cout) {
  if (N <= 0 || h <= 0 || w <= 0 || Cx <= 0 || Cout <= 0) return 0;
  size_t m = 0;
  for (const bool b16 : {false, true}) {
    WgradCall c;
    c.taps = true; c.b16 = b16;
    c.N = N; c.H = h; c.W = w; c.Cx = Cx; c.Cout = Cout;
    const size_t f = wgrad_ws_floats(c, wgrad_select(c, 0));
    if (f > m) m = f;
  }
  return m * sizeof(float);
}

static int up_bwd_weight_impl(const WgradCall& c, hipStream_t stream) {
  UNET_REQUIRE(c.x && c.dy && c.dw && c.workspace, "conv3x3_up_bwd_weight: null pointer");
  UNET_REQUIRE(c.Cx > 0 && c.Cx % 32 == 0 && c.Cout > 0 && c.Cout % 32 == 0 && c.N > 0 && c.H > 0 &&
                   c.W > 0,
               "conv3x3_up_bwd_weight: bad shape Cx=%d Cout=%d", c.Cx, c.Cout);
  UNET_REQUIRE(c.ci_offset >= 0 && c.ci_offset + c.Cx <= c.Cin_total, "conv3x3_up_bwd_weight: bad ci slice");
  UNET_REQUIRE(!c.alpha || c.beta, "conv3x3_up_bwd_weight: alpha without beta");
  const WgradSel sel = wgrad_select(c, 0);
  UNET_REQUIRE(sel.nmax >= 1, "conv3x3_up_bwd_weight: one image exceeds the 2 GiB buffer-descriptor range");
  const size_t need = wgrad_ws_floats(c, sel) * sizeof(float);
  if (c.workspace_bytes < need) {
    unet_set_error("conv3x3_up_bwd_weight: workspace %zu < %zu bytes", c.workspace_bytes, need);
    return UNET_E_WORKSPACE;
  }
  float* ws = reinterpret_cast<float*>(c.workspace);
  int nslab = 0;
  const int rc = wgrad_launch_chunks(c, sel, ws, &nslab, stream);
  if (rc != UNET_OK) return rc;
  return emit_wgrad_reduction(ws, nslab, (size_t)9 * c.Cx * c.Cout, c.dw, c.Cx, c.Cout, c.ci_offset,
                              c.Cin_total, false, false, stream);
}

extern "C" int unet_conv3x3_up_bwd_weight(const unet_act_src* x, float slope, const float* D,
                                          float* dw_oihw, int ci_offset, int Cin_total,
                                          void* workspace, size_t workspace_bytes, int N, int h,
                                          int w, int Cout, unet_stream_t stream) {
  WgradCall c;
  set_source(c, x, slope);
  c.dy = D; c.taps = true;
  c.dw = dw_oihw; c.ci_offset = ci_offset; c.Cin_total = Cin_total;
  c.workspace = workspace; c.workspace_bytes = workspace_bytes;
  c.N = N; c.H = h; c.W = w; c.Cout = Cout;
  return up_bwd_weight_impl(c, (hipStream_t)stream);
}

extern "C" int unet_conv3x3_up_bwd_weight_b16(const unet_act_src* x, float slope, const uint16_t* D,
                                              float* dw_oihw, int ci_offset, int Cin_total,
                                              void* workspace, size_t workspace_bytes, int N,
                                              int h, int w, int Cout, unet_stream_t stream) {
  WgradCall c;
  set_source(c, x, slope);
  c.dy = D; c.taps = true; c.b16 = true;
  c.dw = dw_oihw; c.ci_offset = ci_offset; c.Cin_total = Cin_total;
  c.workspace = workspace; c.workspace_bytes = workspace_bytes;
  c.N = N; c.H = h; c.W = w; c.Cout = Cout;
  return up_bwd_weight_impl(c, (hipStream_t)stream);
}

extern "C" int unet_wgrad_defer_begin(void) {
  ReduceQueue& q = reduce_queue();
  UNET_REQUIRE(!q.on || q.pending == 0, "wgrad_defer_begin: reductions still pending (flush first)");
  q.on = true;
  return UNET_OK;
}
extern "C" int unet_wgrad_defer_pending(void) { return reduce_queue().pending; }
extern "C" int unet_wgrad_defer_flush(unet_stream_t stream) {
  return flush_reduce_queue((hipStream_t)stream);
}
extern "C" int unet_wgrad_defer_end(unet_stream_t stream) {
  const int rc = flush_reduce_queue((hipStream_t)stream);
  reduce_queue().on = false;
  return rc;
}
```

unet-implementations_amd/csrc/misc.hip:

```cpp
#include "conv_params.h"

#include <cxxabi.h>
#include <stdlib.h>
#include <string.h>

#include <mutex>
#include <string>
#include <vector>

static thread_local char g_err[512] = "";

void unet_set_error(const char* fmt, ...) {
  va_list ap;
  va_start(ap, fmt);
  vsnprintf(g_err, sizeof(g_err), fmt, ap);
  va_end(ap);
}

extern "C" const char* unet_last_error(void) { return g_err; }

namespace unet_conv {
long long& chunk_limit_bytes() {
  static long long lim = (1LL << 31) - 1;
  return lim;
// ... 286 lines not shown
    f32x4 v[3][3][2];
#pragma unroll
    for (int ky = 0; ky < 3; ++ky) {
      int yy = i - 1 + ky;
      yy = yy < 0 ? 0 : (yy > h - 1 ? h - 1 : yy);
#pragma unroll
      for (int kx = 0; kx < 3; ++kx) {
        int xx = j - 1 + kx;
        xx = xx < 0 ? 0 : (xx > w - 1 ? w - 1 : xx);
        const bf16x8 q = *reinterpret_cast<const bf16x8*>(b + ((size_t)yy * w + xx) * C);
#pragma unroll
        for (int k = 0; k < 4; ++k) { v[ky][kx][0][k] = (float)q[k]; v[ky][kx][1][k] = (float)q[4 + k]; }
        if (alpha) {
          v[ky][kx][0] = unet_conv::act4(v[ky][kx][0], al[0], be[0], slope, true);
          v[ky][kx][1] = unet_conv::act4(v[ky][kx][1], al[1], be[1], slope, true);
        }
      }
    }
    const float wy[2][2] = {{i > 0 ? 0.25f : 0.f, i > 0 ? 0.75f : 1.f}, {0.75f, 0.25f}};
    const float wx[2][2] = {{j > 0 ? 0.25f : 0.f, j > 0 ? 0.75f : 1.f}, {0.75f, 0.25f}};
    __bf16* o = y + (((size_t)n * 2 * h + 2 * i) * W2 + 2 * j) * C + c;
#pragma unroll
    for (int a = 0; a < 2; ++a)
#pragma unroll
      for (int bb = 0; bb < 2; ++bb) {
        bf16x8 out;
#pragma unroll
        for (int hf = 0; hf < 2; ++hf) {
          const f32x4 res = blend2x2(v[a][bb][hf], v[a][bb + 1][hf], v[a + 1][bb][hf],
                                                v[a + 1][bb + 1][hf], wx[bb][0], wx[bb][1],
                                                wy[a][0], wy[a][1]);
#pragma unroll
          for (int k = 0; k < 4; ++k) out[4 * hf + k] = (__bf16)res[k];
        }
        *reinterpret_cast<bf16x8*>(o + ((size_t)a * W2 + bb) * C) = out;
      }
  }
}

__device__ __forceinline__ int bwd_taps(int i, int n_in, int idx[4], float wt[4]) {
  const int L = n_in - 1;
  int k = 0;
  idx[k] = 2 * i;     wt[k] = (i == 0) ? 1.0f : 0.75f; ++k;
  idx[k] = 2 * i + 1; wt[k] = (i == L) ? 1.0f : 0.75f; ++k;
  if (i >= 1) { idx[k] = 2 * i - 1; wt[k] = 0.25f; ++k; }
  if (i < L)  { idx[k] = 2 * i + 2; wt[k] = 0.25f; ++k; }
  return k;
}

__global__ __launch_bounds__(256) void upsample2x_bwd_kernel(const float* __restrict__ gy,
                                                             float* gx, int h, int w, int C,
                                                             long long total4, int accumulate) {
  const int lpp = C >> 2;
  const int W2 = 2 * w;
  const long long stride = (long long)gridDim.x * 256;
  for (long long i = (long long)blockIdx.x * 256 + threadIdx.x; i < total4; i += stride) {
    const long long pix = i / lpp;
    const int c = (int)(i - pix * lpp) * 4;
    const int ix = (int)(pix % w);
    const long long r = pix / w;
    const int iy = (int)(r % h);
    const long long n = r / h;
    int ys[4], xs[4];
    float wy[4], wx[4];
    const int ny = bwd_taps(iy, h, ys, wy), nx = bwd_taps(ix, w, xs, wx);
    const float* b = gy + (size_t)n * (4 * (size_t)h * w) * C + c;
    f32x4 acc = {0.f, 0.f, 0.f, 0.f};
    for (int a = 0; a < ny; ++a) {
      f32x4 row = {0.f, 0.f, 0.f, 0.f};
      for (int q = 0; q < nx; ++q)
        row += *reinterpret_cast<const f32x4*>(b + ((size_t)ys[a] * W2 + xs[q]) * C) * wx[q];
      acc += row * wy[a];
    }
    f32x4* o = reinterpret_cast<f32x4*>(gx + i * 4);
    if (accumulate) acc += *o;
    *o = acc;
  }
}

template <typename TS, int V = 1>
__global__ __launch_bounds__(256) void upsample2x_bwd_taps_kernel(const TS* __restrict__ dy,
                                                                  TS* __restrict__ D, int h,
                                                                  int w, int C, long long total4) {
  const int lpp = C / (4 * V);
  const int H2 = 2 * h, W2 = 2 * w;
  const long long stride = (long long)gridDim.x * 256;
  for (long long i4 = (long long)blockIdx.x * 256 + threadIdx.x; i4 < total4; i4 += stride) {
    const long long pix = i4 / lpp;
    const int c = (int)(i4 - pix * lpp) * 4 * V;
    const int j = (int)(pix % w);
    const long long r = pix / w;
    const int i = (int)(r % h);
    const long long n = r / h;
    float wy[4], wx[4];
    wy[0] = i >= 1 ? 0.25f : 0.f;
    wy[1] = i == 0 ? 1.0f : 0.75f;
    wy[2] = i == h - 1 ? 1.0f : 0.75f;
    wy[3] = i < h - 1 ? 0.25f : 0.f;
    wx[0] = j >= 1 ? 0.25f : 0.f;
    wx[1] = j == 0 ? 1.0f : 0.75f;
    wx[2] = j == w - 1 ? 1.0f : 0.75f;
    wx[3] = j < w - 1 ? 0.25f : 0.f;
    const TS* b = dy + (size_t)n * H2 * W2 * C + c;
    f32x4 acc[3][3][V];
#pragma unroll
    for (int ky = 0; ky < 3; ++ky)
#pragma unroll
      for (int kx = 0; kx < 3; ++kx)
#pragma unroll
        for (int q = 0; q < V; ++q) acc[ky][kx][q] = f32x4{0.f, 0.f, 0.f, 0.f};
#pragma unroll
    for (int rr = 0; rr < 6; ++rr) {
      const int Ry = 2 * i - 2 + rr;
      if ((unsigned)Ry >= (unsigned)H2) continue;
      f32x4 v[6][V];
#pragma unroll
      for (int cc = 0; cc < 6; ++cc) {
        const int Rx = 2 * j - 2 + cc;
        const bool in = (unsigned)Rx < (unsigned)W2;
        if constexpr (V == 2) {
          bf16x8 q8 = {};
          if (in) q8 = *reinterpret_cast<const bf16x8*>(b + ((size_t)Ry * W2 + Rx) * C);
#pragma unroll
          for (int k = 0; k < 4; ++k) { v[cc][0][k] = (float)q8[k]; v[cc][1][k] = (float)q8[4 + k]; }
        } else {
          v[cc][0] = in ? ld4(b + ((size_t)Ry * W2 + Rx) * C) : f32x4{0.f, 0.f, 0.f, 0.f};
        }
      }
      f32x4 colsum[3][V];
#pragma unroll
      for (int kx = 0; kx < 3; ++kx) {
#pragma unroll
        for (int q = 0; q < V; ++q) {
          f32x4 t = {0.f, 0.f, 0.f, 0.f};
#pragma unroll
          for (int bb = 0; bb < 4; ++bb) {
            const int S = 2 * j - 1 + bb;
            const float wgt = (unsigned)S < (unsigned)W2 ? wx[bb] : 0.f;
            t += v[bb + 2 - kx][q] * wgt;
          }
          colsum[kx][q] = t;
        }
      }
#pragma unroll
      for (int ky = 0; ky < 3; ++ky) {
        const int a = rr + ky - 2;
        if (a < 0 || a > 3) continue;
        const int R = 2 * i - 1 + a;
        const float wgt = (unsigned)R < (unsigned)H2 ? wy[a] : 0.f;
#pragma unroll
        for (int kx = 0; kx < 3; ++kx)
#pragma unroll
          for (int q = 0; q < V; ++q) acc[ky][kx][q] += colsum[kx][q] * wgt;
      }
    }
    TS* o = D + (size_t)pix * 9 * C + c;
#pragma unroll
    for (int ky = 0; ky < 3; ++ky)
#pragma unroll
      for (int kx = 0; kx < 3; ++kx) {
        if constexpr (V == 2) {
          bf16x8 out;
#pragma unroll
          for (int k = 0; k < 4; ++k) {
            out[k] = (__bf16)acc[ky][kx][0][k];
            out[4 + k] = (__bf16)acc[ky][kx][1][k];
          }
          *reinterpret_cast<bf16x8*>(o + (size_t)(ky * 3 + kx) * C) = out;
        } else {
          st4(o + (size_t)(ky * 3 + kx) * C, acc[ky][kx][0]);
        }
      }
  }
}

__global__ __launch_bounds__(256) void resize_bilinear_fwd_kernel(const float* __restrict__ x,
                                                                  float* __restrict__ y, int h,
                                                                  int w, int H, int W,
                                                                  long long total) {
  const float sy = (float)h / (float)H, sx = (float)w / (float)W;
  const long long stride = (long long)gridDim.x * 256;
  for (long long i = (long long)blockIdx.x * 256 + threadIdx.x; i < total; i += stride) {
    const int X = (int)(i % W);
    const long long r = i / W;
    const int Y = (int)(r % H);
    const long long pl = r / H;
    int y0, y1, x0, x1;
    float ly, lx;
    bil_src(Y, sy, h, y0, y1, ly);
    bil_src(X, sx, w, x0, x1, lx);
    const float* p = x + pl * (long long)h * w;
    const float top = (1.f - lx) * p[(size_t)y0 * w + x0] + lx * p[(size_t)y0 * w + x1];
    const float bot = (1.f - lx) * p[(size_t)y1 * w + x0] + lx * p[(size_t)y1 * w + x1];
    y[i] = (1.f - ly) * top + ly * bot;
  }
}
__device__ __forceinline__ void bil_range(int i, float scale, int out, int& lo, int& hi) {
  const float inv = 1.f / scale;
  lo = (int)floorf(((float)i - 0.5f) * inv - 0.5f) - 1;
  hi = (int)ceilf(((float)i + 1.5f) * inv - 0.5f) + 1;
  lo = lo < 0 ? 0 : lo;
  hi = hi > out - 1 ? out - 1 : hi;
}
__device__ __forceinline__ float bil_coef(int dst, float scale, int in, int i) {
  int i0, i1;
  float l;
  bil_src(dst, scale, in, i0, i1, l);
  float c = 0.f;
  if (i0 == i) c += 1.f - l;
  if (i1 == i) c += l;
  return c;
}
__global__ __launch_bounds__(256) void resize_bilinear_bwd_kernel(const float* __restrict__ gy,
                                                                  float* __restrict__ gx, int h,
                                                                  int w, int H, int W,
                                                                  long long total) {
  const float sy = (float)h / (float)H, sx = (float)w / (float)W;
  const long long stride = (long long)gridDim.x * 256;
  for (long long i = (long long)blockIdx.x * 256 + threadIdx.x; i < total; i += stride) {
    const int ix = (int)(i % w);
    const long long r = i / w;
    const int iy = (int)(r % h);
    const long long pl = r / h;
    int ylo, yhi, xlo, xhi;
    bil_range(iy, sy, H, ylo, yhi);
    bil_range(ix, sx, W, xlo, xhi);
    const float* g = gy + pl * (long long)H * W;
    float acc = 0.f;
    for (int Y = ylo; Y <= yhi; ++Y) {
      const float cy = bil_coef(Y, sy, h, iy);
      if (cy == 0.f) continue;
      float row = 0.f;
      for (int X = xlo; X <= xhi; ++X) {
        const float cx = bil_coef(X, sx, w, ix);
        if (cx != 0.f) row += cx * g[(size_t)Y * W + X];
      }
      acc += cy * row;
    }
    gx[i] = acc;
  }
}

__global__ __launch_bounds__(256) void sgd_nesterov_kernel(float* __restrict__ p,
// ... 75 lines not shown
                     (hipStream_t)stream, w, reinterpret_cast<__bf16*>(wf3),
                     reinterpret_cast<__bf16*>(wd3), Cout, Cin);
  UNET_CHECK_LAUNCH("pack_w_split");
  return UNET_OK;
}

extern "C" int unet_pack_conv3x3_weights_batched(const unet_pack_entry* table_device, int n,
                                                 int total_tiles, unet_stream_t stream) {
  UNET_REQUIRE(table_device && n > 0 && n <= 256 && total_tiles > 0,
               "pack_conv3x3_weights_batched: bad argument");
  hipLaunchKernelGGL(pack_w_batched_kernel, dim3((unsigned)total_tiles), dim3(256), 0,
                     (hipStream_t)stream, table_device, n);
  UNET_CHECK_LAUNCH("pack_w_batched");
  return UNET_OK;
}

extern "C" int unet_upsample2x_fwd(const float* x, float* y, int N, int h, int w, int C,
                                   unet_stream_t stream) {
  UNET_REQUIRE(x && y && N > 0 && h > 0 && w > 0 && C > 0 && C % 4 == 0,
               "upsample2x_fwd: bad argument");
  const long long total4 = (long long)N * 4 * h * w * (C / 4);
  hipLaunchKernelGGL(upsample2x_fwd_kernel<float>, dim3(stream_grid(total4)), dim3(256), 0,
                     (hipStream_t)stream, x, y, h, w, C, total4, (const float*)nullptr,
                     (const float*)nullptr, 0.f);
  UNET_CHECK_LAUNCH("upsample2x_fwd");
  return UNET_OK;
}

extern "C" int unet_upsample2x_in_fwd(const unet_act_src* x, float slope, float* up, int N, int h,
                                      int w, unet_stream_t stream) {
  UNET_REQUIRE(x && x->x && up && N > 0 && h > 0 && w > 0 && x->C > 0 && x->C % 4 == 0 &&
                   (!x->alpha || x->beta),
               "upsample2x_in_fwd: bad argument");
  const long long total4 = (long long)N * 4 * h * w * (x->C / 4);
  hipLaunchKernelGGL(upsample2x_fwd_kernel<float>, dim3(stream_grid(total4)), dim3(256), 0,
                     (hipStream_t)stream, x->x, up, h, w, x->C, total4, x->alpha, x->beta, slope);
  UNET_CHECK_LAUNCH("upsample2x_fwd");
  return UNET_OK;
}

extern "C" int unet_upsample2x_in_fwd_b16(const unet_act_src* x, float slope, uint16_t* up, int N,
                                          int h, int w, unet_stream_t stream) {
  UNET_REQUIRE(x && x->x && up && N > 0 && h > 0 && w > 0 && x->C > 0 && x->C % 4 == 0 &&
                   (!x->alpha || x->beta),
               "upsample2x_in_fwd_b16: bad argument");
  if (x->C % 8 == 0) {
    const long long total8 = (long long)N * h * w * (x->C / 8);
    hipLaunchKernelGGL(upsample2x_fwd_b16x8_kernel, dim3(stream_grid(total8)), dim3(256), 0,
                       (hipStream_t)stream, reinterpret_cast<const __bf16*>(x->x),
                       reinterpret_cast<__bf16*>(up), h, w, x->C, total8, x->alpha, x->beta, slope);
    UNET_CHECK_LAUNCH("upsample2x_fwd(b16 x8)");
    return UNET_OK;
  }
  const long long total4 = (long long)N * 4 * h * w * (x->C / 4);
  hipLaunchKernelGGL(upsample2x_fwd_kernel<__bf16>, dim3(stream_grid(total4)), dim3(256), 0,
                     (hipStream_t)stream, reinterpret_cast<const __bf16*>(x->x),
                     reinterpret_cast<__bf16*>(up), h, w, x->C, total4, x->alpha, x->beta, slope);
  UNET_CHECK_LAUNCH("upsample2x_fwd(b16)");
  return UNET_OK;
}

extern "C" int unet_upsample2x_bwd(const float* gy, float* gx, int N, int h, int w, int C,
                                   int accumulate, unet_stream_t stream) {
  UNET_REQUIRE(gy && gx && N > 0 && h > 0 && w > 0 && C > 0 && C % 4 == 0,
               "upsample2x_bwd: bad argument");
  const long long total4 = (long long)N * h * w * (C / 4);
  hipLaunchKernelGGL(upsample2x_bwd_kernel, dim3(stream_grid(total4)), dim3(256), 0,
                     (hipStream_t)stream, gy, gx, h, w, C, total4, accumulate);
  UNET_CHECK_LAUNCH("upsample2x_bwd");
  return UNET_OK;
}

extern "C" int unet_upsample2x_bwd_taps(const float* dy, float* D, int N, int h, int w, int C,
                                        unet_stream_t stream) {
  UNET_REQUIRE(dy && D && N > 0 && h > 0 && w > 0 && C > 0 && C % 4 == 0,
               "upsample2x_bwd_taps: bad argument");
  const long long total4 = (long long)N * h * w * (C / 4);
  hipLaunchKernelGGL(upsample2x_bwd_taps_kernel<float>, dim3(stream_grid(total4)), dim3(256), 0,
                     (hipStream_t)stream, dy, D, h, w, C, total4);
  UNET_CHECK_LAUNCH("upsample2x_bwd_taps");
  return UNET_OK;
}

extern "C" int unet_upsample2x_bwd_taps_b16(const uint16_t* dy, uint16_t* D, int N, int h, int w,
                                            int C, unet_stream_t stream) {
  UNET_REQUIRE(dy && D && N > 0 && h > 0 && w > 0 && C > 0 && C % 4 == 0,
               "upsample2x_bwd_taps_b16: bad argument");
  if (C % 8 == 0) {
    const long long total8 = (long long)N * h * w * (C / 8);
    hipLaunchKernelGGL((upsample2x_bwd_taps_kernel<__bf16, 2>), dim3(stream_grid(total8)), dim3(256),
                       0, (hipStream_t)stream, reinterpret_cast<const __bf16*>(dy),
                       reinterpret_cast<__bf16*>(D), h, w, C, total8);
    UNET_CHECK_LAUNCH("upsample2x_bwd_taps(b16 x8)");
    return UNET_OK;
  }
  const long long total4 = (long long)N * h * w * (C / 4);
  hipLaunchKernelGGL(upsample2x_bwd_taps_kernel<__bf16>, dim3(stream_grid(total4)), dim3(256), 0,
                     (hipStream_t)stream, reinterpret_cast<const __bf16*>(dy),
                     reinterpret_cast<__bf16*>(D), h, w, C, total4);
  UNET_CHECK_LAUNCH("upsample2x_bwd_taps(b16)");
  return UNET_OK;
}

extern "C" int unet_sgd_nesterov_step(float* params, const float* grads, float* momentum,
                                      int64_t n, float lr, float mu, float weight_decay,
                                      int first_step, float grad_scale, unet_stream_t stream) {
  UNET_REQUIRE(params && grads && momentum && n > 0, "sgd_nesterov_step: bad argument");
  UNET_REQUIRE(((uintptr_t)params % 16 == 0) && ((uintptr_t)grads % 16 == 0) &&
                   ((uintptr_t)momentum % 16 == 0),
               "sgd_nesterov_step: arenas must be 16-byte aligned");
  hipLaunchKernelGGL(sgd_nesterov_kernel, dim3(stream_grid((n + 3) / 4)), dim3(256), 0,
                     (hipStream_t)stream, params, grads, momentum, (long long)n, lr, mu,
                     weight_decay, first_step, grad_scale, (const float*)nullptr);
  UNET_CHECK_LAUNCH("sgd_nesterov");
  return UNET_OK;
}

extern "C" int unet_sgd_nesterov_step_dev(float* params, const float* grads, float* momentum,
                                          int64_t n, const float* hyper, int first_step,
                                          unet_stream_t stream) {
  UNET_REQUIRE(params && grads && momentum && hyper && n > 0, "sgd_nesterov_step_dev: bad argument");
  UNET_REQUIRE(((uintptr_t)params % 16 == 0) && ((uintptr_t)grads % 16 == 0) &&
                   ((uintptr_t)momentum % 16 == 0),
               "sgd_nesterov_step_dev: arenas must be 16-byte aligned");
  hipLaunchKernelGGL(sgd_nesterov_kernel, dim3(stream_grid((n + 3) / 4)), dim3(256), 0,
                     (hipStream_t)stream, params, grads, momentum, (long long)n, 0.f, 0.f, 0.f,
                     first_step, 1.f, hyper);
  UNET_CHECK_LAUNCH("sgd_nesterov(dev)");
  return UNET_OK;
}

extern "C" int unet_transpose2d(const float* src, float* dst, int R, int C, unet_stream_t stream) {
  UNET_REQUIRE(src && dst && R > 0 && C > 0, "transpose2d: bad argument");
  hipLaunchKernelGGL(transpose2d_kernel, dim3(ceil_div(C, 32), ceil_div(R, 32)), dim3(256), 0,
                     (hipStream_t)stream, src, dst, R, C);
  UNET_CHECK_LAUNCH("transpose2d");
  return UNET_OK;
}

extern "C" int unet_preprocess_u8(const uint8_t* image_hwc, const uint8_t* mask, float* out_nhwc,
                                  int64_t* target, int N, int H, int W, const float* mean3,
                                  const float* std3, unet_stream_t stream) {
  UNET_REQUIRE(image_hwc && out_nhwc && mean3 && std3 && N > 0 && H > 0 && W > 0 &&
                   (mask == nullptr || target != nullptr),
               "preprocess_u8: bad argument");
  const long long pixels = (long long)N * H * W;
  hipLaunchKernelGGL(preprocess_u8_kernel, dim3(stream_grid(pixels)), dim3(256), 0,
                     (hipStream_t)stream, image_hwc, mask, out_nhwc,
                     reinterpret_cast<long long*>(target), pixels, mean3[0], mean3[1], mean3[2],
                     std3[0], std3[1], std3[2]);
  UNET_CHECK_LAUNCH("preprocess_u8");
  return UNET_OK;
}

extern "C" int unet_resize_bilinear_fwd(const float* x, float* y, int planes, int h, int w, int H,
                                        int W, unet_stream_t stream) {
  UNET_REQUIRE(x && y && planes > 0 && h > 0 && w > 0 && H > 0 && W > 0,
               "resize_bilinear_fwd: bad argument");
  const long long total = (long long)planes * H * W;
  hipLaunchKernelGGL(resize_bilinear_fwd_kernel, dim3(stream_grid(total)), dim3(256), 0,
                     (hipStream_t)stream, x, y, h, w, H, W, total);
  UNET_CHECK_LAUNCH("resize_bilinear_fwd");
  return UNET_OK;
}

extern "C" int unet_resize_bilinear_bwd(const float* gy, float* gx, int planes, int h, int w, int H,
// ... 10 lines not shown
```

unet-implementations_amd/ops.py:

```python
import ctypes
import functools
import struct
import threading

import torch

from ._lib import ActSrc, BwdStats, check, lib


_raw_stream = getattr(torch._C, "_cuda_getCurrentRawStream", None)
_raw_device = getattr(torch._C, "_cuda_getDevice", None)


def _stream():
    if _raw_stream is not None and _raw_device is not None:
        return _raw_stream(_raw_device())
    return torch.cuda.current_stream().cuda_stream


class KernelTimer:

    def __init__(self, only=None):
        self.only = only
        self.records = []
# ... 704 lines not shown
    else:
        assert dw_oihw.shape[0] == Cout and dw_oihw.is_contiguous()
        head = (rx, slope, _ptr(dy), _ptr(dw_oihw), ci_offset, dw_oihw.shape[1], ksize, stride)
    ws = _wgrad_ws(lib().unet_conv3x3_bwd_weight_workspace_bytes(N, H, W, Cx, Cout, stride), dy)
    t0 = _begin("wgrad")
    check(fn(*head, _ptr(ws), ws.numel(), N, H, W, Cout, _stream()))
    if t0 is not None:
        wino = not u8 and not b16 and not x3 and ksize == 3 and \
            bool(lib().unet_conv3x3_bwd_weight_is_winograd(N, H, W, Cx, Cout, stride))
        Ho, Wo = (H, W) if u8 else dy.shape[1:3]
        _end_conv(t0, "conv_stem_wgrad" if Cx == 3 else "conv_wgrad" + sfx,
                  2.0 * N * Ho * Wo * ksize * ksize * Cx * Cout, 2, wino)
    return dw_oihw


def stem_in_bwd_weight_fold_supported(x, g):
    xt = x.x if isinstance(x, (Act, U8Image)) else x
    return g.dtype == torch.float32 and xt.shape[3] == 3 and xt.shape[2] % 128 == 0 and \
        xt.dtype in (torch.float32, torch.uint8) and getattr(x, "alpha", None) is None


def stem_in_bwd_weight_fold(x, g, y, mean, rstd, gamma, beta, mask, slope, partials, dw_oihw,
                            dgamma, dbeta, dbias):
    u8 = isinstance(x, U8Image)
    if not u8 and not isinstance(x, Act):
        x = Act(x)
    N, H, W, _ = x.shape
    Cout = g.shape[3]
    if u8:
        img = (None, _ptr(x.x), *x.c_mean_std())
    else:
        if x.alpha is not None:
            raise ValueError("the RGB image is a plain operand")
        img = (_ptr(x.x), None, None, None)
    ws = _wgrad_ws(lib().unet_stem_in_bwd_weight_fold_workspace_bytes(N, H, W, Cout), g)
    t0 = _begin("wgrad")
    check(lib().unet_stem_in_bwd_weight_fold(
        *img, _ptr(g), _ptr(y), _ptr(mean), _ptr(rstd), _ptr(gamma), _ptr(beta), _ptr(mask), slope,
        _ptr(partials[0]), partials[1], _ptr(dw_oihw), _ptr(dgamma), _ptr(dbeta), _ptr(dbias),
        _ptr(ws), ws.numel(), N, H, W, Cout, _stream()))
    if t0 is not None:
        _end_conv(t0, "conv_stem_wgrad", 2.0 * N * H * W * 27 * Cout, 3, False)
    return dw_oihw


def conv_in_bwd_weight_fold32_supported(x, g):
    xt = x.x if isinstance(x, Act) else x
    if isinstance(x, U8Image) or xt.dtype != torch.float32 or g.dtype != torch.float32 or \
            xt.shape[:3] != g.shape[:3]:
        return False
    N, H, W, Cx = xt.shape
    return bool(lib().unet_conv_in_bwd_weight_fold32_supported(N, H, W, Cx, g.shape[3]))


def conv_in_bwd_weight_fold32(x, slope_x, g, y, mean, rstd, gamma, beta, mask, slope, partials,
                              dw_oihw, ci_offset, dgamma, dbeta, dbias):
    x, rx = _act(x)
    N, H, W, _ = x.shape
    assert dw_oihw.shape[0] == 32 and dw_oihw.is_contiguous() and g.is_contiguous()
    ws = _wgrad_ws(lib().unet_conv_in_bwd_weight_fold32_workspace_bytes(N, H, W), g)
    t0 = _begin("wgrad")
    check(lib().unet_conv_in_bwd_weight_fold32(
        rx, slope_x, _ptr(g), _ptr(y), _ptr(mean), _ptr(rstd), _ptr(gamma), _ptr(beta), _ptr(mask),
        slope, _ptr(partials[0]), partials[1], _ptr(dw_oihw), ci_offset, dw_oihw.shape[1],
        _ptr(dgamma), _ptr(dbeta), _ptr(dbias), _ptr(ws), ws.numel(), N, H, W, _stream()))
    if t0 is not None:
        _end_conv(t0, "conv_wgrad", 2.0 * N * H * W * 9 * 32 * 32, 3, True)
    return g


def upsample2x_in_fwd(x, slope):
    x, rx = _act(x)
    N, h, w, C = x.shape
    b16 = _is_b16(x.x)
    up = (_b16 if b16 else _f32)((N, 2 * h, 2 * w, C), x.x)
    t0 = _begin()
    check(_twin("unet_upsample2x_in_fwd", b16)(rx, slope, _ptr(up), N, h, w, _stream()))
    if t0 is not None:
        _timer.end("upsample2x_fwd", 0.0, 1, t0,
                   nbytes=x.x.element_size() * (x.x.numel() + up.numel()))
    return up


def upsample2x_bwd_taps(dy):
    N, H2, W2, C = dy.shape
    b16 = _is_b16(dy)
    D = (_b16 if b16 else _f32)((N, H2 // 2, W2 // 2, 9 * C), dy)
    t0 = _begin()
    check(_twin("unet_upsample2x_bwd_taps", b16)(_ptr(dy), _ptr(D), N, H2 // 2, W2 // 2, C,
                                                 _stream()))
    if t0 is not None:
        _timer.end("upsample2x_bwd_taps", 0.0, 1, t0,
                   nbytes=dy.element_size() * dy.numel() * (1 + 9 / 4))
    return D


def conv3x3_up_bwd_weight(x, slope, D, dw_oihw, ci_offset):
    x, rx = _act(x)
    N, h, w, Cx = x.shape
    Cout = D.shape[3] // 9
    assert D.shape[:3] == x.shape[:3] and dw_oihw.shape[0] == Cout and dw_oihw.is_contiguous()
    ws = _wgrad_ws(lib().unet_conv3x3_up_bwd_weight_workspace_bytes(N, h, w, Cx, Cout), D)
    b16 = _is_b16(D)
    t0 = _begin("wgrad")
    check(_twin("unet_conv3x3_up_bwd_weight", b16)(
        rx, slope, _ptr(D), _ptr(dw_oihw), ci_offset, dw_oihw.shape[1], _ptr(ws), ws.numel(), N, h,
        w, Cout, _stream()))
    if t0 is not None:
        _end_lowres(t0, "conv_wgrad_bf16" if b16 else "conv_wgrad", N, h, w, Cx, Cout, 2)
    return dw_oihw


@functools.lru_cache(maxsize=None)
def _sel_conv3x3_up_bwd_data(b16, has_wd3, has_nxt):
    wb = b16 and has_wd3
    bs = wb or has_nxt
    return (_export("unet_conv3x3_up_bwd_data" + ("_bs" if bs else "") + ("_b16" if b16 else "") +
                    ("_wb" if wb else "")), wb, bs, "conv_igemm_bf16" if b16 else "conv_igemm")


def conv3x3_up_bwd_data(D, wd, ci_offset, ccols, out=None, accumulate=False, nxt=None, wd3=None):
    N, h, w, C9 = D.shape
    Cout = C9 // 9
    cin_total = wd.shape[1]
    assert wd.shape[0] == 9 and wd.shape[2] == Cout
    b16 = _is_b16(D)
    g = out if out is not None else (_b16 if b16 else _f32)((N, h, w, ccols), D)
    fn, planes, takes_bs, tag = _sel_conv3x3_up_bwd_data(b16, wd3 is not None, nxt is not None)
    w3 = (_ptr(wd3),) if planes else ()
    args = (_ptr(D), _ptr(wd), *w3, cin_total, ci_offset, _ptr(g), N, h, w, Cout, ccols,
            1 if accumulate else 0)
    t0 = _begin("conv")
    if takes_bs:
        _call_nxt(fn, args, nxt)
    else:
        check(fn(*args, _stream()))
    if t0 is not None:
        _end_lowres(t0, tag, N, h, w, ccols, Cout, 1)
    return g


def head1x1_in_fwd(x, slope, w, b):
    x, rx = _act(x)
    N, H, W, C = x.shape
    K = w.shape[0]
    logits = _f32((N, K, H, W), x.x)
    t0 = _begin()
    check(_twin("unet_head1x1_in_fwd", _is_b16(x.x))(rx, slope, _ptr(w), _ptr(b), _ptr(logits), N,
                                                     H * W, K, _stream()))
    if t0 is not None:
        _timer.end("head_fwd", 0.0, 1, t0,
                   nbytes=x.x.element_size() * x.x.numel() + 4.0 * logits.numel())
    return logits


def head1x1_in_bwd(x, slope, dlogits, w, dw, db, nxt=None):
    x, rx = _act(x)
    N, H, W, C = x.shape
    K = w.shape[0]
    da = torch.empty_like(x.x)
    ws = _ws(lib().unet_head1x1_bwd_workspace_bytes(N, H * W, C, K), x.x)
    args = (rx, slope, _ptr(dlogits), _ptr(w), _ptr(da), _ptr(dw), _ptr(db), _ptr(ws), ws.numel(),
            N, H * W, K)
    fn = _twin("unet_head1x1_in_bwd" + ("_bs" if nxt is not None else ""), _is_b16(x.x))
    t0 = _begin()
    if nxt is not None:
        _call_nxt(fn, args, nxt)
    else:
        check(fn(*args, _stream()))
    if t0 is not None:
        _timer.end("head_bwd", 0.0, 2, t0,
                   nbytes=da.element_size() * 2 * da.numel() + 4.0 * dlogits.numel())
    return da


def head1x1_in_bwd_fold(x, slope, dlogits, w, dw, db, nxt, dgamma, dbeta, dbias):
    x, rx = _act(x)
    N, H, W, C = x.shape
    K = w.shape[0]
    dz = torch.empty_like(x.x)
    ws = _ws(lib().unet_head1x1_in_bwd_fold_workspace_bytes(N, H * W, K), x.x)
    t0 = _begin()
    _call_nxt(lib().unet_head1x1_in_bwd_fold,
              (rx, slope, _ptr(dlogits), _ptr(w), _ptr(dz), _ptr(dw), _ptr(db), _ptr(dgamma),
               _ptr(dbeta), _ptr(dbias), _ptr(ws), ws.numel(), N, H * W, K), nxt)
    nxt.applied = nxt.tiles > 0
    if t0 is not None:
        _timer.end("head_bwd", 0.0, 4 if nxt.applied else 2, t0,
                   nbytes=4.0 * ((3 if nxt.applied else 2) * dz.numel() +
                                 (2 if nxt.applied else 1) * dlogits.numel()))
    return dz


def upsample2x_fwd(x):
    N, h, w, C = x.shape
    y = _f32((N, 2 * h, 2 * w, C), x)
    check(lib().unet_upsample2x_fwd(_ptr(x), _ptr(y), N, h, w, C, _stream()))
    return y


def upsample2x_bwd(gy, out=None, accumulate=False):
    N, H2, W2, C = gy.shape
    h, w = H2 // 2, W2 // 2
    gx = out if out is not None else _f32((N, h, w, C), gy)
    check(lib().unet_upsample2x_bwd(_ptr(gy), _ptr(gx), N, h, w, C, 1 if accumulate else 0,
                                    _stream()))
    return gx


def head1x1_fwd(a, w, b):
    N, H, W, C = a.shape
# ... 902 lines not shown
```

unet-implementations_amd/unet.py:

```python
from typing import Dict, List, Optional, Tuple, Type, Union

import torch
import torch.nn as nn

from . import ops


class SpatialDropout2d(nn.Module):

    def __init__(self, drop_prob):
        super().__init__()
        self.drop_prob = drop_prob

    def extra_repr(self):
        return f"drop_prob={self.drop_prob}"

    def draw_mask(self, n, channels, device):
        mask = torch.empty(n, channels, 1, 1, device=device).bernoulli_(1 - self.drop_prob)
        return mask.div_(1 - self.drop_prob).view(n, channels)

    def forward(self, x):
        if not self.training or self.drop_prob == 0:
            return x
        return x * self.draw_mask(x.size(0), x.size(1), x.device).view(x.size(0), x.size(1), 1, 1)
# ... 128 lines not shown
        gx = None
        if g is not None:
            gx = ops.nhwc_to_nchw(ops.upsample2x_bwd(g) if ctx.up else g)
        gskip = ops.nhwc_to_nchw(dx1) if dx1 is not None else None
        return (None, None, gx, gskip, *grads)


def _parse_block(block, first_of_decoder, prefix):
    mods = list(block.block)
    layers, i = [], 0
    while i < len(mods):
        conv = mods[i]
        if not isinstance(conv, nn.Conv2d):
            raise NotImplementedError(f"{prefix}: unexpected module {type(conv).__name__}")
        ks, st = _as_int(conv.kernel_size), _as_int(conv.stride)
        if ks != 3 or st not in (1, 2) or _as_int(conv.padding) != 1 or conv.bias is None \
                or conv.groups != 1 or _as_int(conv.dilation) != 1:
            raise NotImplementedError(
                f"{prefix}.block.{i}: the HIP path covers 3x3/pad 1/stride 1|2 convs with bias")
        i += 1
        norm = mods[i] if i < len(mods) else None
        if not (isinstance(norm, nn.InstanceNorm2d) and norm.affine
                and not norm.track_running_stats):
            raise NotImplementedError(
                f"{prefix}: the HIP path needs InstanceNorm2d(affine=True) after each conv")
        i += 1
        act = mods[i] if i < len(mods) else None
        if not isinstance(act, nn.LeakyReLU):
            raise NotImplementedError(f"{prefix}: the HIP path needs LeakyReLU after the norm")
        i += 1
        drop = None
        if i < len(mods) and isinstance(mods[i], SpatialDropout2d):
            drop = mods[i]
            i += 1
        if i < len(mods) and not isinstance(mods[i], nn.Conv2d):
            raise NotImplementedError(
                f"{prefix}: dropout_op={type(mods[i]).__name__} is not on the HIP path")
        layers.append(_Layer(conv, norm, float(act.negative_slope), drop, st,
                             first_of_decoder and not layers, f"{prefix}.block.{len(layers)}"))
    return layers


class _Layer:

    __slots__ = ("conv", "norm", "slope", "drop", "stride", "first_of_decoder", "name", "ksize")

    def __init__(self, conv, norm, slope, drop, stride, first_of_decoder, name, ksize=3):
        self.conv, self.norm, self.slope, self.drop = conv, norm, slope, drop
        self.stride, self.first_of_decoder, self.name = stride, first_of_decoder, name
        self.ksize = ksize


class _Rec:

    __slots__ = ("layer", "x0", "x1", "low", "y", "st", "mask", "a", "wd", "wd3", "ud", "ud1",
                 "bwd_hooks", "completes", "skip_dst", "nxt")

    def __init__(self, layer, x0, x1, y, st, mask, bwd_forms, place, low=None, a=None):
        self.layer, self.x0, self.x1, self.low, self.a = layer, x0, x1, low, a
        self.y, self.st, self.mask = y, st, mask
        self.wd, self.wd3, self.ud, self.ud1 = bwd_forms
        self.bwd_hooks, self.completes, self.skip_dst = place
        self.nxt = None

    def next_norm(self):
        l = self.layer
        self.nxt = ops.NextNorm(self.y, self.st, l.norm.weight.detach(), l.norm.bias.detach(),
                                self.mask, l.slope)
        return self.nxt

    def output(self):
        return self.a if self.a is not None else ops.Act(self.y, self.st[2], self.st[3])


def _as_int(v):
    if isinstance(v, (tuple, list)):
        if len(set(v)) != 1:
            return None
        return int(v[0])
    return int(v)


class UNet(nn.Module):

    def __init__(self, in_channels: int = 3, num_classes: int = 3, n_stages: int = 6,
                 features_per_stage: List[int] = None,
                 kernel_sizes: List[Tuple[int, int]] = None,
                 strides: List[Tuple[int, int]] = None, n_conv_per_stage: List[int] = None,
                 n_conv_per_stage_decoder: List[int] = None, conv_bias: bool = True,
                 norm_op: Type[nn.Module] = nn.InstanceNorm2d, norm_op_kwargs: Dict = None,
                 dropout_op: Optional[Type[nn.Module]] = None, dropout_op_kwargs: Dict = None,
                 nonlin: Type[nn.Module] = nn.LeakyReLU, nonlin_kwargs: Dict = None,
                 encoder_dropout_rates: List[float] = None,
                 decoder_dropout_rates: List[float] = None):
        super().__init__()
        if features_per_stage is None:
            features_per_stage = [32, 64, 128, 256, 512, 512]
        if kernel_sizes is None:
            kernel_sizes = [[3, 3]] * n_stages
        if strides is None:
            strides = [[1, 1]] + [[2, 2]] * (n_stages - 1)
        if n_conv_per_stage is None:
            n_conv_per_stage = [2] * n_stages
        if n_conv_per_stage_decoder is None:
            n_conv_per_stage_decoder = [2] * (n_stages - 1)
        if norm_op_kwargs is None:
            norm_op_kwargs = {"eps": 1e-5, "affine": True}
        if nonlin_kwargs is None:
            nonlin_kwargs = {"inplace": True}
        if encoder_dropout_rates is None:
            encoder_dropout_rates = [0.0, 0.0, 0.1, 0.2, 0.3, 0.3]
        if decoder_dropout_rates is None:
            decoder_dropout_rates = [0.3, 0.2, 0.2, 0.1, 0.0]

        self.in_channels = in_channels
        self.num_classes = num_classes
        self.n_stages = n_stages
        self.features_per_stage = features_per_stage

        common = dict(norm_op=norm_op, norm_op_kwargs=norm_op_kwargs, dropout_op=dropout_op,
                      dropout_op_kwargs=dropout_op_kwargs, nonlin=nonlin,
                      nonlin_kwargs=nonlin_kwargs, conv_bias=conv_bias)
        self.encoder_stages = nn.ModuleList()
        cin = in_channels
        for s in range(n_stages):
            self.encoder_stages.append(
                ConvBlock(cin, features_per_stage[s], kernel_sizes[s], strides[s],
                          n_convs=n_conv_per_stage[s],
                          spatial_dropout_rate=encoder_dropout_rates[s], **common))
            cin = features_per_stage[s]
        self._fusion_layer = None
        self._build_bottleneck(common)
        self.decoder_stages = nn.ModuleList()
        for s in range(n_stages - 1):
            lvl = n_stages - 2 - s
            self.decoder_stages.append(
                UpBlock(features_per_stage[lvl + 1], features_per_stage[lvl],
                        features_per_stage[lvl], kernel_sizes[lvl],
                        n_convs=n_conv_per_stage_decoder[lvl],
                        spatial_dropout_rate=decoder_dropout_rates[s], **common))
        self._build_head(features_per_stage[0], num_classes)
        self.initialize_weights()
        self._plan = None
        self._arena = None
        self._grad_arena = None
        self._offsets = None
        self.dropout_mask_override = None
        self.grad_ready_hook = None
        self.matmul_precision = "fp32"
        self.fused_pipeline = True
        self.winograd = True
        self.fullres_folds = True
        self.wgrad32_folds = True
        self.input_mean, self.input_std = ops.IMAGENET_MEAN, ops.IMAGENET_STD

    def _build_bottleneck(self, common):
        """Hook for variants that add modules between encoder and decoder (CLIPUNet)."""

    def _build_head(self, in_features, out_channels):
        self.segmentation_output = nn.Conv2d(in_features, out_channels, kernel_size=1, stride=1,
                                             padding=0, bias=True)

    def _head_module(self):
        return self.segmentation_output

    def _check_head(self):
# ... 324 lines not shown
        m = self.mask_of[id(l)]
        y, st = ops.conv_in_fwd(s0, s1, self.slope, w, l.conv.bias.detach(), l.ksize, l.stride,
                                l.norm.weight.detach(), l.norm.bias.detach(), l.norm.eps, m,
                                b16=self.b16, w3=w3, wu=wu)
        return self._fused_output(l, None if low is not None else s0, s1, low, y, st, m,
                                  bwd_forms, place)

    def run_up_layer(self, l, low, skip, place):
        if not self.fused:
            return self.run_layer(l, ops.upsample2x_fwd(low), skip, place)
        if self.x3 or l.ksize != 3 or \
                not ops.conv_up_in_fwd_supported(low, skip, l.conv.weight.shape[0]):
            return self.run_layer_fused(l, ops.Act(ops.upsample2x_in_fwd(low, self.slope)), skip,
                                        place, low=low)
        (w, w3, wu), bwd_forms = self.weight_forms(l, low, skip, up=True)
        m = self.mask_of[id(l)]
        y, st = ops.conv_up_in_fwd(low, skip, self.slope, w, l.conv.bias.detach(),
                                   l.norm.weight.detach(), l.norm.bias.detach(), l.norm.eps, m,
                                   wu=wu, w3=w3)
        return self._fused_output(l, None, skip, low, y, st, m, bwd_forms, place)

    def _fused_output(self, l, x0, x1, low, y, st, m, bwd_forms, place):
        if self.need_grad:
            self.saved.append(_Rec(l, x0, x1, y, st, m, bwd_forms, place, low=low))
        if self.dbg_fwd is not None:
            self.dbg_fwd.append((l.name, y, st))
        return ops.Act(y, st[2], st[3])

    def stage_output(self, v):
        if isinstance(v, ops.Act):
            if v.x.dtype != torch.float32:
                raise NotImplementedError("sub-module hooks on the bf16 pipeline")
            a = v.x if v.alpha is None else ops.instnorm_lrelu_drop_fwd(v.x, v.alpha, v.beta,
                                                                        None, self.slope)
            return ops.nhwc_to_nchw(a)
        return ops.nhwc_to_nchw(v)

    def layer_bwd(self, i, g_a, stop, dx0_acc=None, grad_only=False):
        rec = self.saved[i]
        l, st, x0, x1, low = rec.layer, rec.st, rec.x0, rec.x1, rec.low
        fused, slope = self.fused, self.slope
        gv = (lambda p: None) if grad_only else self.model._grad_view
        need_dx = i > stop
        need_dx1 = rec.skip_dst is not None and rec.skip_dst > stop
        dbg = getattr(self.model, "_debug_capture", None)
        if dbg is not None:
            dbg.append((l.name, "ga", g_a.clone()))
        nn_, rec.nxt = rec.nxt, None
        nxt = self.saved[i - 1].next_norm() \
            if fused and need_dx and not (grad_only and i - 1 == stop) else None
        dw = gv(l.conv.weight)
        want_dw = l.conv.weight.requires_grad and not grad_only
        partials = (nn_.partial, nn_.tiles) if nn_ is not None and nn_.tiles > 0 else None
        if i == 0 and fused and want_dw and partials is not None and dbg is None and \
                self.mode == "fp32" and x1 is None and low is None and l.ksize == 3 and \
                self.model.fullres_folds and ops.stem_in_bwd_weight_fold_supported(x0, g_a):
            ops.stem_in_bwd_weight_fold(x0, g_a, rec.y, st[0], st[1], l.norm.weight.detach(),
                                        l.norm.bias.detach(), rec.mask, l.slope, partials, dw,
                                        gv(l.norm.weight), gv(l.norm.bias), gv(l.conv.bias))
            return None, None
        xw = x1 if low is not None else x0
        fold32 = fused and want_dw and partials is not None and dbg is None and \
            self.mode == "fp32" and not self.x3 and l.ksize == 3 and l.stride == 1 and \
            self.model.wgrad32_folds and not (nn_ is not None and nn_.applied) and \
            (low is not None or x1 is None) and xw is not None and \
            not _hooked(rec.bwd_hooks, "_backward_hooks") and \
            ops.conv_in_bwd_weight_fold32_supported(xw, g_a)
        if nn_ is not None and nn_.applied:
            dy = g_a
        elif fold32:
            dy = ops.conv_in_bwd_weight_fold32(
                xw, slope, g_a, rec.y, st[0], st[1], l.norm.weight.detach(), l.norm.bias.detach(),
                rec.mask, l.slope, partials, dw, low.shape[3] if low is not None else 0,
                gv(l.norm.weight), gv(l.norm.bias), gv(l.conv.bias))
        else:
            dy = ops.instnorm_lrelu_drop_bwd(g_a, rec.y, st[0], st[1], l.norm.weight.detach(),
                                             l.norm.bias.detach(), rec.mask, l.slope,
                                             gv(l.norm.weight), gv(l.norm.bias), gv(l.conv.bias),
                                             partials=partials)
        if dbg is not None:
            dbg.append((l.name, "dy", dy.clone()))
        if low is not None:
            C0 = low.shape[3]
            D = ops.upsample2x_bwd_taps(dy) if (want_dw or need_dx) else None
            if want_dw:
                ops.conv3x3_up_bwd_weight(low, slope, D, dw, 0)
                if not fold32:
                    ops.conv_in_bwd_weight(x1, slope, dy, dw, C0, 3, 1, x3=self.x3)
            g_low = ops.conv3x3_up_bwd_data(D, rec.wd, 0, C0, nxt=nxt,
                                            wd3=rec.wd3 if ops._is_b16(D) else None) \
                if need_dx else None
            dx1 = ops.conv3x3_bwd_data(dy, rec.wd, C0, x1.shape[3], x1.shape[1], x1.shape[2], 1,
                                       wd3=rec.wd3,
                                       bf16="bf16x3" if rec.wd3 is not None else False,
                                       ud=rec.ud1) if need_dx1 else None
            return g_low, dx1
        if want_dw and fused and fold32:
            want_dw = False
        elif want_dw and fused:
            ops.conv_in_bwd_weight(x0, slope, dy, dw, 0, l.ksize, l.stride, x3=self.x3)
            if x1 is not None:
                ops.conv_in_bwd_weight(x1, slope, dy, dw, x0.shape[3], l.ksize, l.stride,
                                       x3=self.x3)
            want_dw = False
        if l.ksize == 1:
            if want_dw:
                dw2d = dw.view(dw.shape[0], dw.shape[1])
                ops.conv1x1_bwd_weight(x0, dy, dw2d, 0)
                if x1 is not None:
                    ops.conv1x1_bwd_weight(x1, dy, dw2d, x0.shape[3])
            dx0 = ops.conv1x1_bwd_data(dy, rec.wd, 0, x0.shape[3]) if need_dx else None
            return dx0, None
        if want_dw:
            ops.conv3x3_bwd_weight(x0, dy, dw, 0, l.stride, bf16=self.mode)
            if x1 is not None:
                ops.conv3x3_bwd_weight(x1, dy, dw, x0.shape[3], l.stride, bf16=self.mode)
        dx0 = dx1 = None
        N, H, W, C0 = x0.shape
        if need_dx:
            dx0 = ops.conv3x3_bwd_data(dy, rec.wd, 0, C0, H, W, l.stride, out=dx0_acc,
                                       accumulate=dx0_acc is not None, bf16=self.mode,
                                       wd3=rec.wd3, nxt=nxt, ud=rec.ud)
        if x1 is not None and need_dx1:
            dx1 = ops.conv3x3_bwd_data(dy, rec.wd, C0, x1.shape[3], H, W, l.stride,
                                       bf16=self.mode, wd3=rec.wd3)
        return dx0, dx1


class _UNetFunction(torch.autograd.Function):
    @staticmethod
    def forward(ctx, model, x, extra, *params):
        c32_mode = "always" if ops.c32_winograd_override() == "always" else bool(model.winograd)
        with ops.c32_winograd_scope(c32_mode):
            logits = _UNetFunction._forward(ctx, model, x, extra, params)
        if any(ctx.needs_input_grad):
            ctx.c32_mode = c32_mode
        return logits

    @staticmethod
    def backward(ctx, dlogits):
        with ops.c32_winograd_scope(ctx.c32_mode), ops.wgrad_deferral() as deferred:
            return _UNetFunction._backward(ctx, dlogits, deferred)

    @staticmethod
    def _forward(ctx, model, x, extra, params, fire_hooks=True):
        fire = _fire_forward_hooks if fire_hooks else (lambda mods, make_output: None)
        enc, dec = model._plan
        fusion = model._fusion_layer if extra is not None else None
        walk = _Walk(model, x, fusion, any(ctx.needs_input_grad))
        fused = walk.fused
        if isinstance(x, ops.U8Image) and not fused:
            raise RuntimeError("the uint8 stem needs the fused pipeline")
        run = walk.run_layer_fused if fused else walk.run_layer
        cur = ops.Act(x) if fused and not isinstance(x, ops.U8Image) else x

        def place(blk, li, hooked, owner, skip_dst=None):
            return (hooked if li == len(blk) - 1 else (), owner if li == 0 else None, skip_dst)

        skips = []
        for bi, blk in enumerate(enc):
            stage = model.encoder_stages[bi]
            for li, l in enumerate(blk):
                cur = run(l, cur, None, place(blk, li, (stage,), stage))
            if bi < len(enc) - 1:
                skips.append((cur, len(walk.saved)))
            fire([stage], lambda: walk.stage_output(cur))
        if fusion is not None:
            if extra.shape[:3] != cur.shape[:3]:
                raise NotImplementedError("bottleneck features must match the 1/32-resolution "
                                          f"grid {tuple(cur.shape[1:3])} (got {tuple(extra.shape[1:3])})")
            cur = run(fusion, cur, ops.Act(extra) if fused else extra,
                      ((), model.clip_fusion_conv, None))
        for di, blk in enumerate(dec):
# ... 129 lines not shown
```

Before: 478.8 images/s.

## Compute only four of nine upsample backward tap planes and redirect reads

In interior pixels of the fused upsample+conv backward, the bilinear-2x tap sums for ky=0 and kx=0 duplicate those of a neighbouring pixel's other taps. The taps kernel now skips computing and storing those redundant planes for fp32 at resolutions of at least 64. The wgrad and dgrad kernels instead redirect their loads to the twin location, which cuts compute and memory traffic in the taps kernel. The cost is extra per-thread index arithmetic and redirect tracking in the igemm and wgrad loaders, plus more complex addressing.

```diff
diff --git a/include/unet_hip.h b/include/unet_hip.h
--- a/include/unet_hip.h
+++ b/include/unet_hip.h
@@ -395,6 +395,16 @@
 int unet_conv3x3_up_bwd_data_bs(const float* D, const float* wd, int Cin_total, int ci_offset,
                                 float* g, int N, int h, int w, int Cout, int Ccols, int accumulate,
                                 unet_bwd_stats* bs, unet_stream_t stream);
+
+int unet_upsample2x_bwd_taps_sparse(const float* dy, float* D, int N, int h, int w, int C,
+                                    unet_stream_t stream);
+int unet_conv3x3_up_bwd_weight_sparse(const unet_act_src* x, float slope, const float* D,
+                                      float* dw_oihw, int ci_offset, int Cin_total,
+                                      void* workspace, size_t workspace_bytes, int N, int h,
+                                      int w, int Cout, unet_stream_t stream);
+int unet_conv3x3_up_bwd_data_sparse(const float* D, const float* wd, int Cin_total, int ci_offset,
+                                    float* g, int N, int h, int w, int Cout, int Ccols,
+                                    int accumulate, unet_bwd_stats* bs, unet_stream_t stream);
 int unet_conv_wino_supported(int N, int H, int W, int C0, int C1, int Cout);
 int unet_set_c32_winograd(int on);
 int unet_conv_c32_is_winograd(int N, int H, int W, int Cin, int Cout, int stride);
diff --git a/unet-implementations_amd/_lib.py b/unet-implementations_amd/_lib.py
--- a/unet-implementations_amd/_lib.py
+++ b/unet-implementations_amd/_lib.py
@@ -181,6 +181,10 @@
     "unet_conv3x3_up_bwd_weight_workspace_bytes": (_sz, [_i, _i, _i, _i, _i]),
     "unet_conv3x3_up_bwd_weight": (_i, [_ps, _f, _p, _p, _i, _i, _p, _sz, _i, _i, _i, _i, _p]),
     "unet_conv3x3_up_bwd_data": (_i, [_p, _p, _i, _i, _p, _i, _i, _i, _i, _i, _i, _p]),
+    "unet_upsample2x_bwd_taps_sparse": (_i, [_p, _p, _i, _i, _i, _i, _p]),
+    "unet_conv3x3_up_bwd_weight_sparse": (_i, [_ps, _f, _p, _p, _i, _i, _p, _sz, _i, _i, _i, _i,
+                                               _p]),
+    "unet_conv3x3_up_bwd_data_sparse": (_i, [_p, _p, _i, _i, _p, _i, _i, _i, _i, _i, _i, _pbs, _p]),
     "unet_head1x1_in_fwd": (_i, [_ps, _f, _p, _p, _p, _i, _i, _i, _p]),
     "unet_head1x1_in_bwd": (_i, [_ps, _f, _p, _p, _p, _p, _p, _p, _sz, _i, _i, _i, _p]),
     "unet_head1x1_in_bwd_bs": (_i, [_ps, _f, _p, _p, _p, _p, _p, _p, _sz, _i, _i, _i, _pbs, _p]),
diff --git a/unet-implementations_amd/csrc/conv_igemm.hip b/unet-implementations_amd/csrc/conv_igemm.hip
--- a/unet-implementations_amd/csrc/conv_igemm.hip
+++ b/unet-implementations_amd/csrc/conv_igemm.hip
@@ -36,9 +36,11 @@
   const int lrow = tid / SEGS, lseg = tid % SEGS;
   int a_nb[A_PASSES], a_iy[A_PASSES], a_ix[A_PASSES];
   int a_img[FUSED ? A_PASSES : 1];
+  unsigned a_red[FUSED ? 1 : A_PASSES];
 #pragma unroll
   for (int i = 0; i < A_PASSES; ++i) {
     const int m = m0 + lrow + ROWS * i;
+    if (!FUSED) a_red[i] = 0u;
     if (m < M) {
       const int n = m / HlWl;
       const int r = m - n * HlWl;
@@ -48,6 +50,8 @@
       a_iy[i] = a * p.sin;
       a_ix[i] = b * p.sin;
       if (FUSED) a_img[i] = n;
+      if (!FUSED && p.taps_sparse)
+        a_red[i] = (a >= 1 && a <= p.Hin - 3 ? 1u : 0u) | (b >= 1 && b <= p.Win - 3 ? 0x10000u : 0u);
     } else {
       a_nb[i] = 0;
       a_iy[i] = -(1 << 24);
@@ -89,6 +93,8 @@
     const __amdgpu_buffer_rsrc_t rs = first ? rs0 : rs1;
     const int Cs = first ? (p.src0_pitch ? p.src0_pitch : p.C0) : p.C1;
     const int coff = (first ? c : c - p.C0) + lseg * 4 + wt * p.tap_cstride;
+    const int red_y = wt < 3 ? p.Win * Cs + 6 * p.tap_cstride : 0;
+    const int red_x = wt % 3 == 0 ? Cs + 2 * p.tap_cstride : 0;
     if (FUSED) {
       const float* al = first ? p.act0_alpha : p.act1_alpha;
       const float* be = first ? p.act0_beta : p.act1_beta;
@@ -114,8 +120,9 @@
       const int iy = a_iy[i] + oy, ix = a_ix[i] + ox;
       const bool ok = (unsigned)iy < (unsigned)p.Hin && (unsigned)ix < (unsigned)p.Win;
       if (FUSED) okm |= (ok ? 1u : 0u) << i;
-      const unsigned off = ((unsigned)((a_nb[i] + iy * p.Win + ix) * Cs + coff) * 4u) |
-                           (ok ? 0u : 0x80000000u);
+      int el = (a_nb[i] + iy * p.Win + ix) * Cs + coff;
+      if (!FUSED) el += (int)(a_red[i] & 0xffffu) * red_y + (int)(a_red[i] >> 16) * red_x;
+      const unsigned off = ((unsigned)el * 4u) | (ok ? 0u : 0x80000000u);
       const i32x4 v = __builtin_amdgcn_raw_buffer_load_b128(rs, off, 0, 0);
       ra[i] = __builtin_bit_cast(f32x4, v);
     }
@@ -1593,9 +1600,11 @@
 static int conv3x3_up_bwd_data_impl(const void* D, const float* wd, int Cin_total, int ci_offset,
                                     void* g, int N, int h, int w, int Cout, int Ccols,
                                     int accumulate, const ConvMode& m, unet_bwd_stats* bs,
-                                    hipStream_t stream) {
+                                    hipStream_t stream, bool taps_sparse = false) {
   if (bs) bs->tiles_out = 0;
   UNET_REQUIRE(D && wd && g, "conv3x3_up_bwd_data: null pointer");
+  UNET_REQUIRE(!taps_sparse || (!m.b16_tensors() && h >= 4 && w >= 4),
+               "conv3x3_up_bwd_data_sparse: needs fp32 tensors and h, w >= 4 (%d x %d)", h, w);
   UNET_REQUIRE(Cout > 0 && Cout % 32 == 0 && Ccols > 0 && Ccols % 32 == 0 && ci_offset >= 0 &&
                    ci_offset + Ccols <= Cin_total && N > 0 && h > 0 && w > 0,
                "conv3x3_up_bwd_data: bad shape Cout=%d Ccols=%d slice %d of %d", Cout, Ccols,
@@ -1607,6 +1616,7 @@
     BsBinder bsb(b.whole(bs), true, N, h * w, Ccols);
     IgemmParams p = dgrad_params(D, wd, Cin_total, ci_offset, g, b, h, w, Cout, Ccols, 1, 3,
                                  accumulate, true, m);
+    p.taps_sparse = taps_sparse ? 1 : 0;
     bsb.bind(p);
     const int rc = m.b16_tensors() ? dispatch_igemm_b16(p, stream, nullptr, bsb.report())
                                    : dispatch_igemm(p, stream, nullptr, bsb.report());
@@ -1627,6 +1637,14 @@
                                         int Ccols, int accumulate, unet_stream_t stream) {
   return conv3x3_up_bwd_data_impl(D, wd, Cin_total, ci_offset, g, N, h, w, Cout, Ccols, accumulate,
                                   ConvMode::f32(), nullptr, (hipStream_t)stream);
+}
+
+extern "C" int unet_conv3x3_up_bwd_data_sparse(const float* D, const float* wd, int Cin_total,
+                                               int ci_offset, float* g, int N, int h, int w,
+                                               int Cout, int Ccols, int accumulate,
+                                               unet_bwd_stats* bs, unet_stream_t stream) {
+  return conv3x3_up_bwd_data_impl(D, wd, Cin_total, ci_offset, g, N, h, w, Cout, Ccols, accumulate,
+                                  ConvMode::f32(), bs, (hipStream_t)stream, true);
 }
 
 extern "C" int unet_conv3x3_up_bwd_data_b16(const uint16_t* D, const float* wd, int Cin_total,
diff --git a/unet-implementations_amd/csrc/conv_params.h b/unet-implementations_amd/csrc/conv_params.h
--- a/unet-implementations_amd/csrc/conv_params.h
+++ b/unet-implementations_amd/csrc/conv_params.h
@@ -33,6 +33,7 @@
   int stats_tiles;
   int tap_cstride;
   int src0_pitch;
+  int taps_sparse;
   const float* bs_y;
   const float* bs_mean;
   const float* bs_rstd;
diff --git a/unet-implementations_amd/csrc/conv_wgrad.hip b/unet-implementations_amd/csrc/conv_wgrad.hip
--- a/unet-implementations_amd/csrc/conv_wgrad.hip
+++ b/unet-implementations_amd/csrc/conv_wgrad.hip
@@ -30,6 +30,7 @@
   const float* beta;
   float slope;
   int b16;
+  int taps_sparse;
   const float* fy; const float* fmu; const float* frstd; const float* fgamma; const float* fbeta;
   const float* fmask; const float2* fcoef; const float2* fsums;
   float* fdgamma; float* fdbeta; float* fdbias;
@@ -292,19 +293,49 @@
   const __amdgpu_buffer_rsrc_t rsd = __builtin_amdgcn_make_buffer_rsrc(
       const_cast<float*>(p.dy), 0, (int)p.dy_bytes, 0x00020000);
 
+  constexpr bool kTapSlots = std::is_same<TD, float>::value;
+  static_assert(!kTapSlots || (NLB == 9 && S * (CO_T / 4) == NT), "one pixel x nine taps per thread");
   int a_px[NLA];
-  unsigned b_off[NLB];
+  unsigned b_off[kTapSlots ? 1 : NLB];
   const int a_ch = ci0 + (tid % (CI_T / 4)) * 4;
 #pragma unroll
   for (int k = 0; k < NLA; ++k) a_px[k] = (tid + NT * k) / (CI_T / 4);
-#pragma unroll
-  for (int k = 0; k < NLB; ++k) {
-    const int idx = tid + NT * k;
-    const int px = idx / (BW / 4);
-    const int f = (idx - px * (BW / 4)) * 4;
-    const int t = f / CO_T;
-    b_off[k] = (unsigned)(px * (9 * p.Cout) + t * p.Cout + co0 + (f - t * CO_T));
-  }
+  const int d_px = tid / (CO_T / 4), d_c = (tid % (CO_T / 4)) * 4;
+  const int d_lds = d_px * BW + d_c;
+  if constexpr (kTapSlots) {
+    b_off[0] = (unsigned)(d_px * (9 * p.Cout) + co0 + d_c);
+  } else {
+#pragma unroll
+    for (int k = 0; k < NLB; ++k) {
+      const int idx = tid + NT * k;
+      const int px = idx / (BW / 4);
+      const int f = (idx - px * (BW / 4)) * 4;
+      const int t = f / CO_T;
+      b_off[k] = (unsigned)(px * (9 * p.Cout) + t * p.Cout + co0 + (f - t * CO_T));
+    }
+  }
+  const int twin_y = kTapSlots && p.taps_sparse ? p.W * 9 * p.Cout + 6 * p.Cout : 0;
+  const int twin_x = kTapSlots && p.taps_sparse ? 9 * p.Cout + 2 * p.Cout : 0;
+  const int d_pr = (d_px / p.W) % p.H, d_pc = d_px % p.W;
+  const int seg_dr = (S / p.W) % p.H, seg_dc = S % p.W;
+  int seg_i = 0, seg_j = 0;
+  unsigned red_y = 0, red_x = 0;
+  auto seg_redirects = [&]() {
+    int j = seg_j + d_pc;
+    const int cy = j >= p.W ? 1 : 0;
+    j -= cy ? p.W : 0;
+    int i = seg_i + d_pr + cy;
+    i -= i >= p.H ? p.H : 0;
+    red_y = i >= 1 && i <= p.H - 3 ? (unsigned)twin_y : 0u;
+    red_x = j >= 1 && j <= p.W - 3 ? (unsigned)twin_x : 0u;
+  };
+  auto seg_advance = [&]() {
+    seg_j += seg_dc;
+    const int cy = seg_j >= p.W ? 1 : 0;
+    seg_j -= cy ? p.W : 0;
+    seg_i += seg_dr + cy;
+    seg_i -= seg_i >= p.H ? p.H : 0;
+  };
 
   f32x4 ra[NLA], rb[NLB];
   f32x4 ca[NLA], cb[NLA];
@@ -324,7 +355,14 @@
       }
     } else {
       constexpr int j = k - NLA;
-      rb[j] = buf_ld4<TD>(rsd, (unsigned)(lq0 * (9 * p.Cout)) + b_off[j], 0u);
+      if constexpr (kTapSlots) {
+        unsigned off = (unsigned)(lq0 * (9 * p.Cout) + j * p.Cout) + b_off[0];
+        if constexpr (j < 3) off += red_y;
+        if constexpr (j % 3 == 0) off += red_x;
+        rb[j] = buf_ld4<TD>(rsd, off, 0u);
+      } else {
+        rb[j] = buf_ld4<TD>(rsd, (unsigned)(lq0 * (9 * p.Cout)) + b_off[j], 0u);
+      }
     }
   };
   auto act_slot = [&](auto kc) {
@@ -338,7 +376,8 @@
       if (NA4 % NT == 0 || tid < NA4) *reinterpret_cast<f32x4*>(base + 4 * (tid + NT * k)) = ra[k];
 #pragma unroll
     for (int k = 0; k < NLB; ++k)
-      *reinterpret_cast<f32x4*>(base + ATILE + 4 * (tid + NT * k)) = rb[k];
+      *reinterpret_cast<f32x4*>(base + ATILE + (kTapSlots ? d_lds + k * CO_T : 4 * (tid + NT * k))) =
+          rb[k];
   };
 
   f32x16 acc[9];
@@ -353,13 +392,25 @@
 
   if (g_begin < g_end) {
     lq0 = g_begin * S;
+    if constexpr (kTapSlots) {
+      const int r0 = lq0 / p.W;
+      seg_j = lq0 - r0 * p.W;
+      seg_i = r0 % p.H;
+      seg_redirects();
+    }
     for_range<0, NLS>(issue_slot);
     for_range<0, NLA>(act_slot);
     store_stage(0);
     __syncthreads();
     for (int g = g_begin; g < g_end; ++g) {
       const int buf = (g - g_begin) & 1;
-      if (g + 1 < g_end) lq0 += S;
+      if (g + 1 < g_end) {
+        lq0 += S;
+        if constexpr (kTapSlots) {
+          seg_advance();
+          seg_redirects();
+        }
+      }
       okm = 0;
       const float* A = smem + buf * STAGE + wi * 32 + li;
       const float* B = smem + buf * STAGE + ATILE + wj * 32 + li;
@@ -2348,6 +2399,7 @@
   int prec = 0;
   bool center_only = false;
   bool taps = false;
+  bool taps_sparse = false;
   float* dw = nullptr;
   int ci_offset = 0, Cin_total = 0;
   float* db = nullptr;
@@ -2440,6 +2492,7 @@
     p.alpha = c.alpha ? c.alpha + (size_t)nb * c.Cx : nullptr;
     p.beta = c.alpha ? c.beta + (size_t)nb * c.Cx : nullptr;
     p.slope = c.slope;
+    p.taps_sparse = c.taps_sparse ? 1 : 0;
     if (c.fold32) {
       UNET_REQUIRE(s.form == WF_WINO32 && nc == c.N, "conv_in_bwd_weight_fold32: not a shape of "
                    "the 32-channel Winograd weight gradient");
@@ -2852,6 +2905,8 @@
                "conv3x3_up_bwd_weight: bad shape Cx=%d Cout=%d", c.Cx, c.Cout);
   UNET_REQUIRE(c.ci_offset >= 0 && c.ci_offset + c.Cx <= c.Cin_total, "conv3x3_up_bwd_weight: bad ci slice");
   UNET_REQUIRE(!c.alpha || c.beta, "conv3x3_up_bwd_weight: alpha without beta");
+  UNET_REQUIRE(!c.taps_sparse || (!c.b16 && c.H >= 4 && c.W >= 4),
+               "conv3x3_up_bwd_weight_sparse: needs fp32 tensors and h, w >= 4 (%d x %d)", c.H, c.W);
   const WgradSel sel = wgrad_select(c, 0);
   UNET_REQUIRE(sel.nmax >= 1, "conv3x3_up_bwd_weight: one image exceeds the 2 GiB buffer-descriptor range");
   const size_t need = wgrad_ws_floats(c, sel) * sizeof(float);
@@ -2880,6 +2935,19 @@
   return up_bwd_weight_impl(c, (hipStream_t)stream);
 }
 
+extern "C" int unet_conv3x3_up_bwd_weight_sparse(const unet_act_src* x, float slope, const float* D,
+                                                 float* dw_oihw, int ci_offset, int Cin_total,
+                                                 void* workspace, size_t workspace_bytes, int N,
+                                                 int h, int w, int Cout, unet_stream_t stream) {
+  WgradCall c;
+  set_source(c, x, slope);
+  c.dy = D; c.taps = true; c.taps_sparse = true;
+  c.dw = dw_oihw; c.ci_offset = ci_offset; c.Cin_total = Cin_total;
+  c.workspace = workspace; c.workspace_bytes = workspace_bytes;
+  c.N = N; c.H = h; c.W = w; c.Cout = Cout;
+  return up_bwd_weight_impl(c, (hipStream_t)stream);
+}
+
 extern "C" int unet_conv3x3_up_bwd_weight_b16(const unet_act_src* x, float slope, const uint16_t* D,
                                               float* dw_oihw, int ci_offset, int Cin_total,
                                               void* workspace, size_t workspace_bytes, int N,
diff --git a/unet-implementations_amd/csrc/misc.hip b/unet-implementations_amd/csrc/misc.hip
--- a/unet-implementations_amd/csrc/misc.hip
+++ b/unet-implementations_amd/csrc/misc.hip
@@ -392,6 +392,8 @@
 __global__ __launch_bounds__(256) void upsample2x_bwd_taps_kernel(const TS* __restrict__ dy,
                                                                   TS* __restrict__ D, int h,
                                                                   int w, int C, long long total4) {
+  const bool sparse = h < 0;
+  if (sparse) h = -h;
   const int lpp = C / (4 * V);
   const int H2 = 2 * h, W2 = 2 * w;
   const long long stride = (long long)gridDim.x * 256;
@@ -411,6 +413,8 @@
     wx[1] = j == 0 ? 1.0f : 0.75f;
     wx[2] = j == w - 1 ? 1.0f : 0.75f;
     wx[3] = j < w - 1 ? 0.25f : 0.f;
+    const bool skip_y = sparse && i >= 1 && i <= h - 3;
+    const bool skip_x = sparse && j >= 1 && j <= w - 3;
     const TS* b = dy + (size_t)n * H2 * W2 * C + c;
     f32x4 acc[3][3][V];
 #pragma unroll
@@ -423,11 +427,12 @@
     for (int rr = 0; rr < 6; ++rr) {
       const int Ry = 2 * i - 2 + rr;
       if ((unsigned)Ry >= (unsigned)H2) continue;
+      if (rr == 5 && skip_y) continue;
       f32x4 v[6][V];
 #pragma unroll
       for (int cc = 0; cc < 6; ++cc) {
         const int Rx = 2 * j - 2 + cc;
-        const bool in = (unsigned)Rx < (unsigned)W2;
+        const bool in = (unsigned)Rx < (unsigned)W2 && !(cc == 5 && skip_x);
         if constexpr (V == 2) {
           bf16x8 q8 = {};
           if (in) q8 = *reinterpret_cast<const bf16x8*>(b + ((size_t)Ry * W2 + Rx) * C);
@@ -440,6 +445,7 @@
       f32x4 colsum[3][V];
 #pragma unroll
       for (int kx = 0; kx < 3; ++kx) {
+        if (kx == 0 && skip_x) continue;
 #pragma unroll
         for (int q = 0; q < V; ++q) {
           f32x4 t = {0.f, 0.f, 0.f, 0.f};
@@ -456,12 +462,15 @@
       for (int ky = 0; ky < 3; ++ky) {
         const int a = rr + ky - 2;
         if (a < 0 || a > 3) continue;
+        if (ky == 0 && skip_y) continue;
         const int R = 2 * i - 1 + a;
         const float wgt = (unsigned)R < (unsigned)H2 ? wy[a] : 0.f;
 #pragma unroll
-        for (int kx = 0; kx < 3; ++kx)
+        for (int kx = 0; kx < 3; ++kx) {
+          if (kx == 0 && skip_x) continue;
 #pragma unroll
           for (int q = 0; q < V; ++q) acc[ky][kx][q] += colsum[kx][q] * wgt;
+        }
       }
     }
     TS* o = D + (size_t)pix * 9 * C + c;
@@ -469,6 +478,7 @@
     for (int ky = 0; ky < 3; ++ky)
 #pragma unroll
       for (int kx = 0; kx < 3; ++kx) {
+        if ((ky == 0 && skip_y) || (kx == 0 && skip_x)) continue;
         if constexpr (V == 2) {
           bf16x8 out;
 #pragma unroll
@@ -710,6 +720,17 @@
   return UNET_OK;
 }
 
+extern "C" int unet_upsample2x_bwd_taps_sparse(const float* dy, float* D, int N, int h, int w,
+                                               int C, unet_stream_t stream) {
+  UNET_REQUIRE(dy && D && N > 0 && h >= 4 && w >= 4 && C > 0 && C % 4 == 0,
+               "upsample2x_bwd_taps_sparse: bad argument (needs h, w >= 4)");
+  const long long total4 = (long long)N * h * w * (C / 4);
+  hipLaunchKernelGGL(upsample2x_bwd_taps_kernel<float>, dim3(stream_grid(total4)), dim3(256), 0,
+                     (hipStream_t)stream, dy, D, -h, w, C, total4);
+  UNET_CHECK_LAUNCH("upsample2x_bwd_taps_sparse");
+  return UNET_OK;
+}
+
 extern "C" int unet_upsample2x_bwd_taps_b16(const uint16_t* dy, uint16_t* D, int N, int h, int w,
                                             int C, unet_stream_t stream) {
   UNET_REQUIRE(dy && D && N > 0 && h > 0 && w > 0 && C > 0 && C % 4 == 0,
diff --git a/unet-implementations_amd/ops.py b/unet-implementations_amd/ops.py
--- a/unet-implementations_amd/ops.py
+++ b/unet-implementations_amd/ops.py
@@ -810,28 +810,47 @@
     return up
 
 
-def upsample2x_bwd_taps(dy):
+def taps_sparse_supported(t, h, w):
+    return t.dtype == torch.float32 and h >= 4 and w >= 4
+
+
+def taps_sparse_kept(h, w, device=None):
+    i = torch.arange(h, device=device).view(h, 1, 1)
+    j = torch.arange(w, device=device).view(1, w, 1)
+    t = torch.arange(9, device=device).view(1, 1, 9)
+    drop = ((t // 3 == 0) & (i >= 1) & (i <= h - 3)) | ((t % 3 == 0) & (j >= 1) & (j <= w - 3))
+    return ~drop
+
+
+def upsample2x_bwd_taps(dy, sparse=False, out=None):
     N, H2, W2, C = dy.shape
     b16 = _is_b16(dy)
-    D = (_b16 if b16 else _f32)((N, H2 // 2, W2 // 2, 9 * C), dy)
-    t0 = _begin()
-    check(_twin("unet_upsample2x_bwd_taps", b16)(_ptr(dy), _ptr(D), N, H2 // 2, W2 // 2, C,
-                                                 _stream()))
+    h, w = H2 // 2, W2 // 2
+    if sparse and not taps_sparse_supported(dy, h, w):
+        raise ValueError(f"upsample2x_bwd_taps: no sparse form for {dy.dtype} at {h} x {w}")
+    D = out if out is not None else (_b16 if b16 else _f32)((N, h, w, 9 * C), dy)
+    assert D.shape == (N, h, w, 9 * C) and D.dtype == dy.dtype
+    fn = lib().unet_upsample2x_bwd_taps_sparse if sparse else _twin("unet_upsample2x_bwd_taps", b16)
+    t0 = _begin()
+    check(fn(_ptr(dy), _ptr(D), N, h, w, C, _stream()))
     if t0 is not None:
         _timer.end("upsample2x_bwd_taps", 0.0, 1, t0,
-                   nbytes=dy.element_size() * dy.numel() * (1 + 9 / 4))
+                   nbytes=dy.element_size() * dy.numel() * (1 + (4 if sparse else 9) / 4))
     return D
 
 
-def conv3x3_up_bwd_weight(x, slope, D, dw_oihw, ci_offset):
+def conv3x3_up_bwd_weight(x, slope, D, dw_oihw, ci_offset, sparse=False):
     x, rx = _act(x)
     N, h, w, Cx = x.shape
     Cout = D.shape[3] // 9
     assert D.shape[:3] == x.shape[:3] and dw_oihw.shape[0] == Cout and dw_oihw.is_contiguous()
     ws = _wgrad_ws(lib().unet_conv3x3_up_bwd_weight_workspace_bytes(N, h, w, Cx, Cout), D)
     b16 = _is_b16(D)
+    if sparse and not taps_sparse_supported(D, h, w):
+        raise ValueError(f"conv3x3_up_bwd_weight: no sparse form for {D.dtype} at {h} x {w}")
     t0 = _begin("wgrad")
-    check(_twin("unet_conv3x3_up_bwd_weight", b16)(
+    check((lib().unet_conv3x3_up_bwd_weight_sparse if sparse
+           else _twin("unet_conv3x3_up_bwd_weight", b16))(
         rx, slope, _ptr(D), _ptr(dw_oihw), ci_offset, dw_oihw.shape[1], _ptr(ws), ws.numel(), N, h,
         w, Cout, _stream()))
     if t0 is not None:
@@ -847,7 +866,8 @@
                     ("_wb" if wb else "")), wb, bs, "conv_igemm_bf16" if b16 else "conv_igemm")
 
 
-def conv3x3_up_bwd_data(D, wd, ci_offset, ccols, out=None, accumulate=False, nxt=None, wd3=None):
+def conv3x3_up_bwd_data(D, wd, ci_offset, ccols, out=None, accumulate=False, nxt=None, wd3=None,
+                        sparse=False):
     N, h, w, C9 = D.shape
     Cout = C9 // 9
     cin_total = wd.shape[1]
@@ -855,6 +875,10 @@
     b16 = _is_b16(D)
     g = out if out is not None else (_b16 if b16 else _f32)((N, h, w, ccols), D)
     fn, planes, takes_bs, tag = _sel_conv3x3_up_bwd_data(b16, wd3 is not None, nxt is not None)
+    if sparse:
+        if not taps_sparse_supported(D, h, w):
+            raise ValueError(f"conv3x3_up_bwd_data: no sparse form for {D.dtype} at {h} x {w}")
+        fn, takes_bs = lib().unet_conv3x3_up_bwd_data_sparse, True
     w3 = (_ptr(wd3),) if planes else ()
     args = (_ptr(D), _ptr(wd), *w3, cin_total, ci_offset, _ptr(g), N, h, w, Cout, ccols,
             1 if accumulate else 0)
diff --git a/unet-implementations_amd/unet.py b/unet-implementations_amd/unet.py
--- a/unet-implementations_amd/unet.py
+++ b/unet-implementations_amd/unet.py
@@ -234,6 +234,9 @@
 
 
 class UNet(nn.Module):
+
+    sparse_taps = True
+    TAPS_SPARSE_MIN_HW = 64
 
     def __init__(self, in_channels: int = 3, num_classes: int = 3, n_stages: int = 6,
                  features_per_stage: List[int] = None,
@@ -724,13 +727,16 @@
             dbg.append((l.name, "dy", dy.clone()))
         if low is not None:
             C0 = low.shape[3]
-            D = ops.upsample2x_bwd_taps(dy) if (want_dw or need_dx) else None
+            hl, wl = low.shape[1], low.shape[2]
+            sp = self.model.sparse_taps and ops.taps_sparse_supported(dy, hl, wl) and \
+                min(hl, wl) >= self.model.TAPS_SPARSE_MIN_HW
+            D = ops.upsample2x_bwd_taps(dy, sparse=sp) if (want_dw or need_dx) else None
             if want_dw:
-                ops.conv3x3_up_bwd_weight(low, slope, D, dw, 0)
+                ops.conv3x3_up_bwd_weight(low, slope, D, dw, 0, sparse=sp)
                 if not fold32:
                     ops.conv_in_bwd_weight(x1, slope, dy, dw, C0, 3, 1, x3=self.x3)
             g_low = ops.conv3x3_up_bwd_data(D, rec.wd, 0, C0, nxt=nxt,
-                                            wd3=rec.wd3 if ops._is_b16(D) else None) \
+                                            wd3=rec.wd3 if ops._is_b16(D) else None, sparse=sp) \
                 if need_dx else None
             dx1 = ops.conv3x3_bwd_data(dy, rec.wd, C0, x1.shape[3], x1.shape[1], x1.shape[2], 1,
                                        wd3=rec.wd3,
```

After: 483.3 images/s, median of 6. About the same (+0.9%).
